# hy-vision-learning/jck-generation

Hardware: AMD Instinct MI355X
Metric: images/sec (G+D step) DCGAN 64x64 bs256 (higher is better)
Workload: dtype bf16; 1 GPU; DCGAN 64x64x3 synthetic, batch 256 per GPU, full G+D step incl. GP pass, RNG and Adam (BASELINE.json configs[1]); per_gpu_batch=256, global_batch=256, parallelism=dp1, dead_D_wgrad_in_G_phase=skipped (never observable: zeroed at train/dcgan_trainer.py:155)

## Files before the change

include/jckgan.h:

```cpp
#ifndef JCKGAN_H
#define JCKGAN_H
#include <stddef.h>
#include <stdint.h>
#ifdef __cplusplus
extern "C" {
#endif

#define JCK_PREC_BF16 0
#define JCK_PREC_F32 1
#define JCK_PREC_BF16X3 2

#define JCK_OK 0
#define JCK_E_ARG (-1)
#define JCK_E_HIP (-2)
#define JCK_E_WS (-3)

const char* jck_last_error(void);
const char* jck_last_launch(void);
const char* jck_launch_name(int i);
int jck_version(void);
int jck_pad_rows(int c);
int jck_pad_chan(int c);

size_t jck_packed_bytes(int prec, long long elems);
int jck_pack_down(int prec, const float* w, int Cs, int Cb, void* wp, void* stream);
int jck_pack_up(int prec, const float* w, int Cs, int Cb, void* wp, void* stream);
int jck_pack_g1(int prec, const float* w, int Ci, int Co, int CiPad, void* wp, void* stream);
int jck_pack_head(const float* w, int C, float* wp, void* stream);

size_t jck_stats_floats(long long pixels, int C, int nyrep);
int jck_conv_down(int prec, const void* big, const void* w, void* small_out, float* stats, int* stats_slots,
                  int N, int Hb, int Wb, int Cb, int Cs, void* stream);
int jck_conv_up(int prec, const void* small_in, const void* w, void* big_out, float* stats, int* stats_slots,
                int epi_tanh, int N, int Hs, int Ws, int Cs, int Cb, void* stream);
size_t jck_conv_wgrad_ws_bytes(int N, int Hb, int Wb, int Cb, int Cs);
int jck_conv_wgrad(int prec, const void* small_side, const void* big_side, float* ws, size_t ws_bytes, float* grad,
                   int accumulate, int N, int Hb, int Wb, int Cb, int Cs, void* stream);
int jck_g1_fwd(int prec, const void* z, const void* w, void* out, float* stats, int* stats_slots, int B, int CiPad,
               int Co, void* stream);
int jck_conv_up_affine(int prec, const void* small_in, const void* w, const float* scale, const float* shift, void* big_out,
                       int N, int Hs, int Ws, int Cs, int Cb, void* stream);
int jck_g1_fwd_affine(int prec, const void* z, const void* w, const float* scale, const float* shift, void* out, int B,
                      int CiPad, int Co, void* stream);
int jck_conv_down_mask(int prec, const void* big, const void* w, const void* a_small, const float* scale, void* small_out,
                       int N, int Hb, int Wb, int Cb, int Cs, void* stream);
int jck_conv_down_affine(int prec, const void* big, const void* w, const float* scale, const float* shift, float slope,
                         void* small_out, int N, int Hb, int Wb, int Cb, int Cs, void* stream);
int jck_latent_loss(int prec, const void* x_nhwc4, const float* target_nchw_f32, void* g_raw_out, float* loss_out, int N, int HW,
                    void* stream);
int jck_latent_adam(int prec, const float* slab, int Z, int ld, float* z, float* m, float* v, float lr, float prior, int t,
                    void* z_operand, int CiPad, int N, void* stream);
int jck_conv_up_mask(int prec, const void* small_in, const void* w, const void* a_big, const float* scale, float slope, void* big_out,
                     int N, int Hs, int Ws, int Cs, int Cb, void* stream);
int jck_leaky_affine_bwd(int prec, const void* g, const void* a, const float* scale, float slope, void* g_y, long long rows, int C,
                         void* stream);
int jck_critic_ds(const float* logit, int mode, float weight, int B, float* ds, float* term, void* stream);
int jck_latent_loss_ex(int prec, const void* x_nhwc4, const float* target_nchw_f32, const float* weight, const void* g_x, void* g_raw_out,
                       float* loss_out, int N, int HW, void* stream);
size_t jck_g1_wgrad_ws_bytes(int B, int CiPad, int Co);
int jck_g1_wgrad(int prec, const void* z, const void* dy, float* ws, size_t ws_bytes, float* grad, int accumulate, int B,
                 int Ci, int CiPad, int Co, void* stream);

int jck_bn_finalize(const float* stats, int slots, float count, const float* gamma, const float* beta,
                    float* running_mean, float* running_var, int64_t* num_batches_tracked, float momentum, float eps,
                    float* aux, int C, void* stream);
int jck_bn_act_fwd(int prec, const void* y, const float* aux, float slope, void* a, long long rows, int C, void* stream);
int jck_bn_eval_aux(int nlayers, const float* const* gamma, const float* const* beta, const float* const* running_mean,
                    const float* const* running_var, float* const* aux, const int* C, float eps, void* stream);
size_t jck_bn_bwd_ws_floats(int C);
int jck_bn_act_bwd(int prec, const void* g_a, const void* y, const float* aux, float slope, float* sums, void* g_y,
                   float* dgamma, float* dbeta, long long rows, int C, void* stream);
int jck_bn_finalize_grouped(const float* stats, int slots_per_group, float count, const float* gamma, const float* beta, float eps,
                            float* aux, float* stat_out, int C, int groups, void* stream);
int jck_bn_fwd(int prec, const void* y, const float* stats, int slots_per_group, float count, const float* gamma, const float* beta,
               float eps, float slope, void* a, float* aux, float* stat_out, float* running_mean, float* running_var, int64_t* nbt,
               float momentum, long long rows_per_group, int C, int groups, void* stream);
int jck_bn_act_fwd_grouped(int prec, const void* y, const float* aux, float slope, void* a, long long rows_per_group, int C,
                           int groups, void* stream);
int jck_bn_act_bwd_grouped(int prec, const void* g_a, const void* y, const float* aux, float slope, float* sums, void* g_y,
                           float* dgamma, float* dbeta, long long rows_per_group, int C, int groups, int grad_groups, void* stream);
size_t jck_grid_sync_bytes(void);
int jck_grid_sync_error(const void* sync_ws);
int jck_bn_act_bwd_res(int prec, const void* g_a, const void* y, const float* aux, float slope, float* sums, void* g_y,
                       float* dgamma, float* dbeta, long long rows_per_group, int C, int groups, int grad_groups, void* sync_ws,
                       void* stream);
int jck_conv_down_grouped(int prec, const void* big, const void* w, void* small_out, float* stats, int* stats_slots, int N, int Hb,
                          int Wb, int Cb, int Cs, int group_images, void* stream);
int jck_conv_up_grouped(int prec, const void* small_in, const void* w, void* big_out, float* stats, int* stats_slots, int N, int Hs,
                        int Ws, int Cs, int Cb, int group_images, void* stream);
int jck_img_prep(int prec, const float* img_nchw, const float* noise_nchw, float keep, float mix, void* out, int N, int HW,
                 void* stream);
int jck_img_prep_u8(int prec, const unsigned char* data, const int64_t* idx, const float* noise, float keep, float mix,
                    void* out_nhwc4, float* out_nchw, int B, int Hs, int Ws, void* stream);
int jck_resize_norm(const float* in, float* out, int N, int C, int H, int W, int OH, int OW, float pre_scale, float pre_shift,
                    const float* mean, const float* stdv, void* stream);
int jck_nhwc4_to_nchw(int prec, const void* in, float* out_nchw, int N, int HW, void* stream);
int jck_img_to_u8(int prec, const void* in, unsigned char* out_u8_nhwc, int N, int HW, void* stream);
int jck_axpy_noise(int prec, const void* x, const float* noise_nchw, float keep, float mix, void* out, int N, int HW,
                   void* stream);
int jck_interp(int prec, const void* a, const void* b, const float* alpha, void* out, int N, int HW, void* stream);
int jck_mix_interp(int prec, const void* x, const float* noise_nchw, const unsigned* rng, int tensor_id, float keep, float mix, void* out,
                   const void* real, const float* alpha, void* xhat, int N, int HW, void* stream);
int jck_gp_norm(int prec, const void* g, int N, int HW, float* scal, int slot, int scal_ld, float* norms, void* stream);
int jck_tanh_bwd(int prec, const void* g, const void* y, float scale, void* out, long long numel, void* stream);
int jck_head_fwd(int prec, const void* a4, const float* wp, const float* bias , int B, int K,
                 float target, int mode, float* prob, float* ds, float* scal, int slot_loss, int slot_p, int scal_ld, void* stream);
int jck_score_head(int prec, const void* x, const float* w, const float* bias , int B, int K,
                   float* logit, float* prob , void* stream);
int jck_head_fwd_grouped(int prec, const void* a4, const float* wp, const float* bias, int B, int K, int G, const float* targets,
                         const int* modes, float* prob, float* ds, float* scal, const int* slot_loss, const int* slot_p,
                         int scal_ld, void* stream);
size_t jck_head_bwd_ws_floats(int K);
int jck_head_bwd(int prec, const float* ds, const float* wp, const void* a4, int B, int K, void* g_a4, float* dwp,
                 int accumulate, float* ws, void* stream);
int jck_head_unpack_grad(const float* dwp, int C, float* grad, int accumulate, void* stream);
int jck_head_bwd_conv(int prec, const float* ds, const float* wp, const void* a4, int B, int C, void* g_a4, float* grad,
                      float* ws, void* stream);
int jck_head_bwd_conv2(int prec, const float* ds, const float* wp, const void* a4, int B, int B_more, int C, void* g_a4, float* grad,
                       float* ws, void* stream);

int jck_pack_linear(int prec, const float* w, int N, int K, int rows, int cols, int transpose, int permC, int permHW, void* wp,
                    void* stream);
int jck_linear_fwd(int prec, const void* x, const void* wp, const float* bias, void* out, int B, int Kpad, int N, int NStore,
                   int ksplit, void* stream);
int jck_linear_finish(int prec, const float* slab, int Z, const float* bias, const float* mask, float scale, void* h, void* hd,
                      int B, int N, void* stream);
size_t jck_linear_wgrad_ws_bytes(int B, int Kpad, int N);
int jck_linear_wgrad(int prec, const void* gy, int ldgy, const void* x, int Kpad, float* ws, size_t ws_bytes, float* gradp,
                     int accumulate, int B, int N, void* stream);
int jck_unperm_linear_grad(const float* gp, int N, int K, int ldp, int permC, int permHW, float* grad, int accumulate, void* stream);
int jck_label_embed_fwd(int prec, const int64_t* labels, const float* W, const float* b, float slope, int B, int NI, int NO,
                        void* cbuf, int ld, int col0, float* pre, void* stream);
int jck_label_embed_bwd(int prec, const void* gc, int ld, int col0, const float* pre, const int64_t* labels, float slope, int B,
                        int NI, int NO, float* dW, float* db, void* stream);
int jck_label_embed_fwd_tiled(int prec, const int64_t* labels, const float* W, const float* b, float slope, int B, int NI, int NO,
                              void* cbuf, int ld, int col0, float* pre, int label_period, void* stream);
int jck_label_embed_bwd_tiled(int prec, const void* gc, int ld, int col0, const float* pre, const int64_t* labels, float slope,
                              int B, int NI, int NO, float* dW, float* db, int label_period, void* stream);
int jck_concat_rows(int prec, const void* a4, int K0, void* cbuf, int ld, int B, void* stream);
int jck_split_rows(int prec, const void* gc, int ld, int K0, void* ga4, int B, void* stream);
int jck_dropout(int prec, const void* x, const float* mask, float scale, void* y, long long n, void* stream);
int jck_colsum(int prec, const void* g, int B, int N, int ld, float* db, void* stream);
int jck_sum_vec(const float* x, int n, float* out, void* stream);
int jck_cgan_z(int prec, const float* z, const int64_t* labels, int B, int NZ, int NL, int CiPad, void* out, void* stream);
int jck_gp_grad(int prec, const void* g, const float* norms, float coef, int N, int HW, void* u, void* stream);
int jck_gp_head2(int prec, const void* ughd, const float* w2, const float* prob, int B, int K, float* rs, float* dw2, float* ws,
                 void* stream);
size_t jck_gp_head2_conv_ws_floats(int B);
int jck_gp_head2_conv(int prec, const void* v4, const void* a4, const float* wp, const float* prob, int B, int C, float* rs,
                      void* g_a4, float* grad, float* ws, void* stream);
size_t jck_bn2_ws_floats(int C);
int jck_bn2_vchain(int prec, const void* v, const void* y, const void* gy, const float* aux, const float* s1, const float* gamma,
                   float slope, float* ws, void* u, void* xdir, float* dgamma, long long rows, int C, void* stream);
int jck_bn2_reverse(int prec, const void* ua, const void* y, const void* xdir, const float* aux, const float* gamma,
                    const float* vsums, float slope, float* ws, void* uy, float* dgamma, float* dbeta, long long rows, int C,
                    void* stream);

int jck_adam(float* p, const float* g, float* m, float* v, long long n, double lr, double beta1, double beta2, double eps,
             int step, float grad_scale, void* stream);
int jck_adam_ema(float* p, const float* g, float* m, float* v, float* ema, long long n, double lr, double beta1, double beta2,
                 double eps, int step, float grad_scale, float ema_weight, const unsigned* skip_if, void* stream);

typedef struct jck_engine jck_engine;
int jck_engine_create(jck_engine** out, int family, int prec, int batch);
int jck_engine_create_sized(jck_engine** out, int family, int prec, int batch, int image_size);
#define JCK_ENGINE_GP_BACKWARD 1u
int jck_engine_create_ex(jck_engine** out, int family, int prec, int batch, int image_size, unsigned flags);
int jck_engine_image_size(const jck_engine*);
int jck_engine_num_tensors_of(const jck_engine*, int net);
int jck_engine_tensor_info_of(const jck_engine*, int net, int idx, char* name, int name_cap, int* kind, long long* offset,
                              long long* numel, int* shape4);
long long jck_engine_arena_numel_of(const jck_engine*, int net, int which);
void jck_engine_destroy(jck_engine*);
int jck_engine_num_tensors(int family, int net );
int jck_engine_tensor_info(int family, int net, int idx, char* name, int name_cap, int* kind, long long* offset,
                           long long* numel, int* shape4);
size_t jck_engine_workspace_bytes(const jck_engine*);
long long jck_engine_arena_numel(int family, int net, int which );
int jck_engine_bind(jck_engine*, void* workspace, size_t ws_bytes, float* g_params, float* g_grads, float* g_m, float* g_v,
                    float* g_bn, int64_t* g_nbt, float* d_params, float* d_grads, float* d_m, float* d_v, float* d_bn,
                    int64_t* d_nbt);
int jck_engine_repack(jck_engine*, int net, void* stream);
#define JCK_PHASE_D_LOSS 0
#define JCK_PHASE_D_GP 1
#define JCK_PHASE_D_STEP 2
#define JCK_PHASE_G_LOSS 3
// ... 109 lines not shown
```

jck-generation_amd/csrc/engine.hip:

```cpp
#include <cstdlib>
#include <cstring>
#include <vector>

#include "ops_internal.hpp"
#include "ew_optim.hpp"
#define JCK_BATCHED_DEFAULT 3
struct jck_engine;
#define TT (e->T)

namespace {

struct TensorInfo { const char* name; int kind; long long offset, numel; int shape[4]; };

struct NetLayout {
  std::vector<TensorInfo> t;
  long long n_params = 0, n_bn = 0;
};

constexpr long long ALIGN_F = 64;

void add_param(NetLayout& L, const char* name, int a, int b, int c, int d) {
  TensorInfo ti{name, 0, L.n_params, (long long)a * b * c * d, {a, b, c, d}};
  L.t.push_back(ti);
  L.n_params = (L.n_params + ti.numel + ALIGN_F - 1) / ALIGN_F * ALIGN_F;
// ... 19 lines not shown
Topo make_topo(int S) {
  Topo T = {};
  T.S = S; T.NS = S == 128 ? 5 : 4; T.HW = S * S;
  T.G_C1 = 64 << (T.NS - 1);
  T.FEAT = 16 * T.G_C1;
  for (int i = 0; i < T.NS; ++i) {
    T.D_CS[i] = 64 << i; T.D_CB[i] = i == 0 ? 3 : 32 << i; T.D_HB[i] = S >> i;
    T.G_CS[i] = T.G_C1 >> i; T.G_CB[i] = i == T.NS - 1 ? 3 : T.G_C1 >> (i + 1); T.G_HS[i] = 4 << i;
  }
  return T;
}
const int N_CLASS = 100, EMB = 200, L1_OUT = 256, L1_FEAT = 8192, L1_K = L1_FEAT + EMB, L1_KPAD = 8448;
constexpr int L1_KSPLIT = 12;
inline int z_dim(int family) { return family == 1 ? 200 : 100; }
inline int z_pad(int family) { return family == 1 ? 256 : 128; }

static const char* const CWN[6] = {"conv1.weight", "conv2.weight", "conv3.weight", "conv4.weight", "conv5.weight", "conv6.weight"};
static const char* const NWN[5] = {"norm1.weight", "norm2.weight", "norm3.weight", "norm4.weight", "norm5.weight"};
static const char* const NBN[5] = {"norm1.bias", "norm2.bias", "norm3.bias", "norm4.bias", "norm5.bias"};
static const char* const RMN[5] = {"norm1.running_mean", "norm2.running_mean", "norm3.running_mean", "norm4.running_mean", "norm5.running_mean"};
static const char* const RVN[5] = {"norm1.running_var", "norm2.running_var", "norm3.running_var", "norm4.running_var", "norm5.running_var"};

NetLayout make_layout(int family, int net, int S = 64) {
  NetLayout L;
  const Topo T = make_topo(S);
  const char* const* CW = CWN; const char* const* NW = NWN; const char* const* NB = NBN; const char* const* RM = RMN; const char* const* RV = RVN;
  if (net == 0) {
    add_param(L, CW[0], z_dim(family), T.G_C1, 4, 4);
    add_bn(L, NW[0], NB[0], RM[0], RV[0], T.G_C1);
    for (int i = 0; i < T.NS; ++i) {
      add_param(L, CW[i + 1], T.G_CS[i], T.G_CB[i], 4, 4);
      if (i < T.NS - 1) add_bn(L, NW[i + 1], NB[i + 1], RM[i + 1], RV[i + 1], T.G_CB[i]);
    }
  } else {
    if (family == 1) {
      add_param(L, "label_embedding.weight", EMB, N_CLASS, 1, 1);
      add_param(L, "label_embedding.bias", EMB, 1, 1, 1);
    }
    for (int i = 0; i < T.NS; ++i) {
      add_param(L, CW[i], T.D_CS[i], T.D_CB[i], 4, 4);
      add_bn(L, NW[i], NB[i], RM[i], RV[i], T.D_CS[i]);
    }
    if (family == 0) {
      add_param(L, CW[T.NS], 1, T.G_C1, 4, 4);
    } else {
      add_param(L, "linear1.weight", L1_OUT, L1_K, 1, 1);
      add_param(L, "linear1.bias", L1_OUT, 1, 1, 1);
      add_param(L, "linear2.weight", 1, L1_OUT, 1, 1);
      add_param(L, "linear2.bias", 1, 1, 1, 1);
    }
  }
  return L;
}

const TensorInfo* find(const NetLayout& L, const char* name) {
  for (auto& t : L.t) if (!strcmp(t.name, name)) return &t;
  return nullptr;
}

struct Carver {
  size_t off = 0;
  unsigned char* base = nullptr;
  template <typename T> T* take(size_t count) {
    T* p = base ? reinterpret_cast<T*>(base + off) : nullptr;
    off = (off + count * sizeof(T) + 255) / 256 * 256;
    return p;
  }
};

struct BnBuf { float *stats, *sums, *aux; int slots; };

struct DActs {
  void *y[JCK_MAX_STAGES], *a[JCK_MAX_STAGES], *g[JCK_MAX_STAGES], *gx;
  float *stats[JCK_MAX_STAGES], *aux[JCK_MAX_STAGES], *sums[JCK_MAX_STAGES], *prob, *ds, *norms;
  int cap, g0, groups;
  DActs group(const jck_engine* e, int first, int n) const;
};

}

static unsigned jck_event_flags() { return hipEventDisableTiming | hipEventDisableSystemFence; }
struct StepState {
  bool gp_done = false;
  bool gp_inflight = false;
  bool join_pending = false, mid_recorded = false;
  long long real_fwd_step = -1;
  bool tail_on_side = false, pre_on_side = false;
  int head_row0 = 0;
  int head_wrow0 = 0;
  int acc_clean_step = -1;
  int dg_clean_step = -1, gg_clean_step = -1;
  long long gz_step = -1;
  void drop_promises() { acc_clean_step = dg_clean_step = gg_clean_step = -1; join_pending = mid_recorded = false; }
  void begin_gp_only() { acc_clean_step = dg_clean_step = -1; gp_done = gp_inflight = false; head_row0 = head_wrow0 = 0; }
};
struct jck_engine {
  int family, prec, B;
  Topo T;
  size_t esz;
  NetLayout LG, LD;
  size_t ws_bytes = 0;
  bool bound = false;
  float *gp = nullptr, *gg = nullptr, *gm = nullptr, *gv = nullptr, *gbn = nullptr;
  float *dp = nullptr, *dg = nullptr, *dm = nullptr, *dv = nullptr, *dbn = nullptr;
  int64_t *gnbt = nullptr, *dnbt = nullptr;
  float* gema = nullptr;
  double ema_decay = 0.0; int ema_start = 0;
  float ema_w(int step) const { return !gema ? 0.f : (step < ema_start ? 1.f : (float)(1.0 - ema_decay)); }
  int graph_nodes = 0;
  void *d_down[JCK_MAX_STAGES], *d_up[JCK_MAX_STAGES];
  float *d_head_wp, *d_head_dwp;
  void *g1_w, *g_up[JCK_MAX_STAGES], *g_down[JCK_MAX_STAGES];
  DActs dset[3] = {};
  DActs bset = {};
  int batched = 0;
  StepState ss;
  float* d_rs[JCK_MAX_STAGES];
  int parity = 0;
  hipStream_t sA = nullptr, sB = nullptr, sC = nullptr;
  hipEvent_t evW[JCK_MAX_STAGES] = {}, evWdone = nullptr, evWmid = nullptr, evHead = nullptr, evTail = nullptr, ev0 = nullptr, evF = nullptr, evReal = nullptr, evGP = nullptr;
  template <typename F> void for_each_side_stream(F f) { for (hipStream_t* p : {&sA, &sB, &sC}) f(*p); }
  template <typename F> void for_each_event(F f) {
    for (hipEvent_t* p : {&evWdone, &evWmid, &evHead, &evTail, &ev0, &evF, &evReal, &evGP}) f(*p);
    for (hipEvent_t& p : evW) f(p);
  }
  bool overlap = true, defer_join = true;
  bool wgrad_side = true;
  bool head_side = true;
  bool ext_events = true;
  unsigned* gsync = nullptr; bool bn_res = true;
  bool cbuf_direct = true;
  bool head_fuse = true;
  bool real_side = true;
  bool fold_zero = true;
  bool fuse_tanh = true;
  void *g_z, *g_y[JCK_MAX_STAGES], *g_a[JCK_MAX_STAGES], *g_gr[JCK_MAX_STAGES], *fake_raw, *fake, *g_raw;
  void *real_noisy, *xhat;
  BnBuf g_bn[JCK_MAX_STAGES];
  float *acc, *scal_out;
  float *acc2, *scal2;
  int acc_ld = 0;
  float *head_ws, *gp2_ws;
  float* hp2;
  unsigned long long noise_seed = 0x6a636b67616e0001ull;
  float *rz[2] = {nullptr, nullptr}, *ralpha[2] = {nullptr, nullptr}, *rmask[2] = {nullptr, nullptr};
  int hp_step[2] = {0, 0};
  float hp_lr[2] = {-1.f, -1.f};
  bool hp_holds(int step, float lr) const { return hp_step[step & 1] == step && hp_lr[step & 1] == lr; }
  bool capturing = false;
  bool gp_bwd = false;
  float* g1_ws = nullptr; size_t g1_ws_bytes = 0;
  float* wg_ws; size_t wg_ws_bytes;
  void *l1_w, *l1_wT;
  void *cbuf, *cbuf2;
  void *h_pre, *h_drop, *g_h, *g_hd, *gh_b1, *ughd, *gc;
  float *pre_e, *l1_slab, *gw1p, *rs, *prob_gp;
  void *d_v[JCK_MAX_STAGES], *d_xdir[JCK_MAX_STAGES], *d_u0;
  float* bn2_ws[JCK_MAX_STAGES]; float* bn2_ws_rev;
  const int64_t* cur_labels = nullptr;
  void* lat_w = nullptr; float *lat_slab = nullptr, *lat_loss = nullptr;
  struct ScoreBufs {
    void* base = nullptr;
    void *x = nullptr, *y = nullptr, *a[JCK_MAX_STAGES] = {}, *cbuf = nullptr, *h = nullptr;
    float *aux[JCK_MAX_STAGES] = {}, *slab = nullptr;
  } sc;
  struct CriticBufs {
    void* base = nullptr;
    void *g[JCK_MAX_STAGES] = {}, *gx = nullptr, *g_h = nullptr, *gc = nullptr;
    float *ds = nullptr, *term = nullptr, *logit = nullptr;
  } cr;
  bool d_packed = false;

  void carve(unsigned char* base) {
    jck_engine* e = this;
    Carver c; c.base = base;
    auto bytes = [&](size_t n) { return n * esz; };
    for (int i = 0; i < TT.NS; ++i) {
      d_down[i] = c.take<unsigned char>(bytes((size_t)jck_pad_rows(TT.D_CS[i]) * 16 * jck_pad_chan(TT.D_CB[i])));
      d_up[i] = c.take<unsigned char>(bytes((size_t)4 * jck_pad_rows(TT.D_CB[i]) * 4 * TT.D_CS[i]));
    }
    d_head_wp = c.take<float>(TT.FEAT); d_head_dwp = c.take<float>(TT.FEAT);
    g1_w = c.take<unsigned char>(bytes((size_t)16 * TT.G_C1 * z_pad(family)));
    for (int i = 0; i < TT.NS; ++i) {
      g_up[i] = c.take<unsigned char>(bytes((size_t)4 * jck_pad_rows(TT.G_CB[i]) * 4 * TT.G_CS[i]));
      g_down[i] = c.take<unsigned char>(bytes((size_t)jck_pad_rows(TT.G_CS[i]) * 16 * jck_pad_chan(TT.G_CB[i])));
    }
    const size_t img = (size_t)B * TT.HW * 4;
    auto take_set = [&](DActs& D, int cap, bool penalty_out) {
      D.cap = D.groups = cap; D.g0 = 0;
      for (int i = 0; i < TT.NS; ++i) {
        const size_t n = (size_t)cap * B * (TT.D_HB[i] / 2) * (TT.D_HB[i] / 2) * TT.D_CS[i];
        D.y[i] = c.take<unsigned char>(bytes(n)); D.a[i] = c.take<unsigned char>(bytes(n)); D.g[i] = c.take<unsigned char>(bytes(n));
        D.sums[i] = c.take<float>(cap * jck_bn_bwd_ws_floats(TT.D_CS[i]));
        D.aux[i] = c.take<float>(cap * 4 * TT.D_CS[i]);
        D.stats[i] = c.take<float>(jck_stats_floats((long long)cap * B * (TT.D_HB[i] / 2) * (TT.D_HB[i] / 2), TT.D_CS[i], 1));
      }
      if (penalty_out) D.gx = c.take<unsigned char>(bytes(img));
      D.prob = c.take<float>((size_t)cap * B); D.ds = c.take<float>((size_t)cap * B);
      if (penalty_out) D.norms = c.take<float>(B);
    };
    for (DActs& D : dset) take_set(D, 1, true);
    for (int i = 0; i < TT.NS; ++i) d_rs[i] = c.take<float>(2 * 4 * 2 * TT.D_CS[i]);
    g_z = c.take<unsigned char>(bytes((size_t)B * z_pad(family)));
    for (int i = 0; i < TT.NS; ++i) {
      const int h = 4 << i, C = TT.G_C1 >> i;
      const size_t n = (size_t)B * h * h * C;
      g_y[i] = c.take<unsigned char>(bytes(n)); g_a[i] = c.take<unsigned char>(bytes(n)); g_gr[i] = c.take<unsigned char>(bytes(n));
    }
    fake_raw = c.take<unsigned char>(bytes(img)); g_raw = c.take<unsigned char>(bytes(img));
    real_noisy = c.take<unsigned char>(bytes(img)); fake = c.take<unsigned char>(bytes(img)); xhat = c.take<unsigned char>(bytes(img));
    if (batched) {
      take_set(bset, 3, false);
      bset.gx = dset[0].gx; bset.norms = dset[0].norms;
    }
    for (int i = 0; i < TT.NS; ++i) g_bn[i].sums = c.take<float>(jck_bn_bwd_ws_floats(TT.G_C1 >> i));
    for (int i = 0; i < TT.NS; ++i) {
      const int C = TT.G_C1 >> i, h = 4 << i;
      g_bn[i].aux = c.take<float>(4 * C);
      g_bn[i].stats = c.take<float>(jck_stats_floats((long long)B * h * h, C, i == 0 ? 16 : 1));
    }
    acc_ld = (B + 63) / 64 * 64;
    acc2 = c.take<float>((size_t)2 * 8 * acc_ld); scal2 = c.take<float>(16);
    acc = acc2; scal_out = scal2;
    hp2 = c.take<float>(16);
    for (int q = 0; q < 2; ++q) {
      rz[q] = c.take<float>((size_t)B * 100); ralpha[q] = c.take<float>((size_t)(B + 3) / 4 * 4);
      rmask[q] = family == 1 ? c.take<float>((size_t)4 * B * L1_OUT) : nullptr;
    }
    head_ws = c.take<float>(jck_head_bwd_ws_floats(TT.FEAT));
    gp2_ws = c.take<float>((size_t)acc_ld + jck_head_bwd_ws_floats(L1_OUT));
    gsync = c.take<unsigned>(jck_grid_sync_bytes() / sizeof(unsigned));
    size_t w = 0;
    for (int i = 0; i < TT.NS; ++i) {
      w = std::max(w, jck_conv_wgrad_ws_bytes(B, TT.D_HB[i], TT.D_HB[i], TT.D_CB[i], TT.D_CS[i]));
      w = std::max(w, jck_conv_wgrad_ws_bytes(2 * B, TT.D_HB[i], TT.D_HB[i], TT.D_CB[i], TT.D_CS[i]));
      w = std::max(w, jck_conv_wgrad_ws_bytes(B, TT.G_HS[i] * 2, TT.G_HS[i] * 2, TT.G_CB[i], TT.G_CS[i]));
    }
    w = std::max(w, jck_g1_wgrad_ws_bytes(B, z_pad(family), TT.G_C1));
    if (family == 1) w = std::max(std::max(w, jck_linear_wgrad_ws_bytes(B, L1_KPAD, L1_OUT)), jck_linear_wgrad_ws_bytes(2 * B, L1_KPAD, L1_OUT));
    wg_ws_bytes = w;
    wg_ws = c.take<float>(w / 4);
    g1_ws_bytes = jck_g1_wgrad_ws_bytes(B, z_pad(family), TT.G_C1);
    g1_ws = c.take<float>(g1_ws_bytes / 4);
    if (family == 1) {
      l1_w = c.take<unsigned char>(bytes((size_t)L1_OUT * L1_KPAD)); l1_wT = c.take<unsigned char>(bytes((size_t)L1_KPAD * L1_OUT));
      const size_t HR = batched ? 3 : 1;
      cbuf = c.take<unsigned char>(bytes(HR * B * L1_KPAD)); cbuf2 = c.take<unsigned char>(bytes((size_t)B * L1_KPAD));
      h_pre = c.take<unsigned char>(bytes(HR * B * L1_OUT)); h_drop = c.take<unsigned char>(bytes(HR * B * L1_OUT));
      g_h = c.take<unsigned char>(bytes(HR * B * L1_OUT)); g_hd = c.take<unsigned char>(bytes(HR * B * L1_OUT));
      gh_b1 = c.take<unsigned char>(bytes((size_t)B * L1_OUT)); ughd = c.take<unsigned char>(bytes((size_t)B * L1_OUT));
      gc = c.take<unsigned char>(bytes(HR * B * L1_KPAD));
      pre_e = c.take<float>(HR * B * EMB); l1_slab = c.take<float>((size_t)L1_KSPLIT * HR * B * L1_OUT);
      gw1p = c.take<float>((size_t)L1_OUT * L1_KPAD);
    }
    if (family == 1 || gp_bwd) {
      rs = c.take<float>(B); prob_gp = c.take<float>(B);
      for (int i = 0; i < TT.NS; ++i) {
        const size_t n = (size_t)B * (TT.D_HB[i] / 2) * (TT.D_HB[i] / 2) * TT.D_CS[i];
        d_v[i] = c.take<unsigned char>(bytes(n)); d_xdir[i] = c.take<unsigned char>(bytes(n));
        bn2_ws[i] = c.take<float>(jck_bn2_ws_floats(TT.D_CS[i]));
      }
      bn2_ws_rev = c.take<float>(jck_bn2_ws_floats(TT.G_C1));
      d_u0 = c.take<unsigned char>(bytes(img));
    }
    ws_bytes = c.off;
  }

  float* P(const NetLayout& L, float* arena, const char* name) const { return arena + find(L, name)->offset; }
  const unsigned* rng() const { return reinterpret_cast<const unsigned*>(hp2 + 8 * parity + 4); }
  int mix_fake_noise(const jck_step_inputs* in, int B, hipStream_t st) {
    if (!in->noise_fake) return jck_axpy_noise_rng(prec, fake_raw, rng(), 1, 0.9f, 0.1f, fake, B, T.HW, st);
    return jck_axpy_noise(prec, fake_raw, in->noise_fake, 0.9f, 0.1f, fake, B, T.HW, st);
  }
  int mix_fake_noise_interp(const jck_step_inputs* in, int B, hipStream_t st) {
    return jck_mix_interp(prec, fake_raw, in->noise_fake, in->noise_fake ? nullptr : rng(), 1, 0.9f, 0.1f, fake, real_noisy, in->alpha, xhat,
                          B, T.HW, st);
  }
};


DActs DActs::group(const jck_engine* e, int first, int n) const {
  DActs v = *this;
  v.g0 = g0 + first; v.groups = n;
  const size_t B = (size_t)e->B;
  auto at = [&](void* p, size_t elems) { return (void*)((unsigned char*)p + elems * e->esz); };
  for (int i = 0; i < TT.NS; ++i) {
    const int cs = TT.D_CS[i];
    const size_t px = (size_t)(TT.D_HB[i] / 2) * (TT.D_HB[i] / 2), off = first * B * px * cs;
    v.y[i] = at(y[i], off); v.a[i] = at(a[i], off); v.g[i] = at(g[i], off);
    v.aux[i] = aux[i] + (size_t)first * 4 * cs;
    v.sums[i] = sums[i] + (size_t)first * jck_bn_bwd_ws_floats(cs);
    v.stats[i] = stats[i] + (size_t)first * (jck_stats_floats((long long)(cap * B * px), cs, 1) / cap / (2 * cs)) * (2 * cs);
  }
  v.prob = prob + first * B; v.ds = ds + first * B;
  return v;
}

static bool env_on(const char* name) {
  const char* v = getenv(name);
  return !(v && atoi(v) == 0);
}
static int create_side_streams(jck_engine* e) {
  hipError_t rc = hipSuccess;
  e->for_each_side_stream([&](hipStream_t& s) { if (rc == hipSuccess) rc = hipStreamCreateWithFlags(&s, hipStreamNonBlocking); });
  e->for_each_event([&](hipEvent_t& ev) { if (rc == hipSuccess) rc = hipEventCreateWithFlags(&ev, jck_event_flags()); });
  HIPCHK(rc);
// ... 215 lines not shown
  return JCK_OK;
}

static int d_head(jck_engine* e, DActs& D, int B, float target, int mode, int slot_loss, int slot_p, hipStream_t st, void* g_out = nullptr) {
  if (e->family == 0)
    return head_fwd_grouped_ev(e->prec, D.a[TT.NS - 1], e->d_head_wp, nullptr, B, TT.FEAT, 1, &target, &mode, D.prob, D.ds, e->acc, &slot_loss,
                               &slot_p, e->acc_ld, g_out, st, nullptr);
  return jck_head_fwd(e->prec, e->h_drop, e->P(e->LD, e->dp, "linear2.weight"), e->P(e->LD, e->dp, "linear2.bias"), B, L1_OUT, target,
                      mode, D.prob, D.ds, e->acc, slot_loss, slot_p, e->acc_ld, st);
}

static int d_head_backward(jck_engine* e, DActs& D, const float* ds, int B, bool want_wgrad, const float* drop_mask, void* ga4_out, hipStream_t st,
                           hipStream_t side = nullptr, bool mid_done = false) {
  if (e->family == 0)
    return jck_head_bwd_conv(e->prec, ds, e->d_head_wp, D.a[TT.NS - 1], B, TT.G_C1, mid_done ? nullptr : ga4_out,
                             want_wgrad ? e->P(e->LD, e->dg, CWN[TT.NS]) : nullptr, e->head_ws, st);
  const size_t r0 = (size_t)e->ss.head_row0, w0 = (size_t)e->ss.head_wrow0;
  auto hb = [&](void* p, size_t row, size_t per_row) { return (void*)((unsigned char*)p + row * per_row * e->esz); };
  void *h_drop = hb(e->h_drop, r0, L1_OUT), *cbuf = hb(e->cbuf, r0, L1_KPAD);
  void *g_hd = hb(e->g_hd, w0, L1_OUT), *g_h = hb(e->g_h, w0, L1_OUT), *gc = hb(e->gc, w0, L1_KPAD);
  const float* pre_e = e->pre_e + r0 * EMB;
  hipStream_t ws = st;
  auto fork = [&](int k) { return fork_side(e, k, st, side, &ws); };
  const float* w2 = e->P(e->LD, e->dp, "linear2.weight");
  if (!mid_done) JCK_TRY(jck_head_bwd(e->prec, ds, w2, h_drop, B, L1_OUT, g_hd, nullptr, 1, e->head_ws, st));
  if (want_wgrad) {
    JCK_TRY(fork(0));
    JCK_TRY(jck_head_bwd(e->prec, ds, w2, h_drop, B, L1_OUT, nullptr, e->P(e->LD, e->dg, "linear2.weight"), 1, e->head_ws, ws));
    JCK_TRY(jck_sum_vec(ds, B, e->P(e->LD, e->dg, "linear2.bias"), ws));
  }
  if (!mid_done) JCK_TRY(jck_dropout(e->prec, g_hd, drop_mask, 1.0f / 0.75f, g_h, (long long)B * L1_OUT, st));
  if (want_wgrad) {
    JCK_TRY(fork(1));
    JCK_TRY(jck_linear_wgrad(e->prec, g_h, L1_OUT, cbuf, L1_KPAD, e->wg_ws, e->wg_ws_bytes, e->gw1p, 1, B, L1_OUT, ws));
    JCK_TRY(jck_colsum(e->prec, g_h, B, L1_OUT, L1_OUT, e->P(e->LD, e->dg, "linear1.bias"), ws));
  }
  JCK_TRY(jck_linear_fwd(e->prec, g_h, e->l1_wT, nullptr, gc, B, L1_OUT, L1_KPAD, L1_KPAD, 1, st));
  if (want_wgrad) {
    JCK_TRY(fork(2));
    JCK_TRY(jck_label_embed_bwd(e->prec, gc, L1_KPAD, TT.FEAT, pre_e, e->cur_labels, LRELU, B, N_CLASS, EMB,
                                e->P(e->LD, e->dg, "label_embedding.weight"), e->P(e->LD, e->dg, "label_embedding.bias"), ws));
  }
  return jck_split_rows(e->prec, gc, L1_KPAD, TT.FEAT, ga4_out, B, st);
}

static int cg_head_backward_batched(jck_engine* e, const float* ds, int B, const float* drop_mask, void* ga4_out, hipStream_t st,
                                    hipStream_t side = nullptr, bool mid_done = false) {
  const int R3 = 3 * B, R2 = 2 * B;
  const float* w2 = e->P(e->LD, e->dp, "linear2.weight");
  hipStream_t ws = st;
  auto fork = [&](int k) { return fork_side(e, k, st, side, &ws); };
  if (!mid_done) JCK_TRY(jck_head_bwd(e->prec, ds, w2, e->h_drop, R3, L1_OUT, e->g_hd, nullptr, 1, e->head_ws, st));
  if (!mid_done) {
    JCK_TRY(fork(0));
    JCK_TRY(jck_head_bwd(e->prec, ds, w2, e->h_drop, R2, L1_OUT, nullptr, e->P(e->LD, e->dg, "linear2.weight"), 1, e->head_ws, ws));
    JCK_TRY(jck_sum_vec(ds, R2, e->P(e->LD, e->dg, "linear2.bias"), ws));
    JCK_TRY(jck_dropout(e->prec, e->g_hd, drop_mask, 1.0f / 0.75f, e->g_h, (long long)R3 * L1_OUT, st));
  }
  JCK_TRY(fork(1));
  if (mid_done) {
    JCK_TRY(jck_head_bwd(e->prec, ds, w2, e->h_drop, R2, L1_OUT, nullptr, e->P(e->LD, e->dg, "linear2.weight"), 1, e->head_ws, ws));
    JCK_TRY(jck_sum_vec(ds, R2, e->P(e->LD, e->dg, "linear2.bias"), ws));
  }
  JCK_TRY(jck_linear_wgrad(e->prec, e->g_h, L1_OUT, e->cbuf, L1_KPAD, e->wg_ws, e->wg_ws_bytes, e->gw1p, 1, R2, L1_OUT, ws));
  JCK_TRY(jck_colsum(e->prec, e->g_h, R2, L1_OUT, L1_OUT, e->P(e->LD, e->dg, "linear1.bias"), ws));
  JCK_TRY(jck_linear_fwd(e->prec, e->g_h, e->l1_wT, nullptr, e->gc, R3, L1_OUT, L1_KPAD, L1_KPAD, 1, st));
  JCK_TRY(fork(2));
  JCK_TRY(jck_label_embed_bwd_tiled(e->prec, e->gc, L1_KPAD, TT.FEAT, e->pre_e, e->cur_labels, LRELU, R2, N_CLASS, EMB,
                                    e->P(e->LD, e->dg, "label_embedding.weight"), e->P(e->LD, e->dg, "label_embedding.bias"), B, ws));
  if (side) HIPCHK(hipEventRecord(e->evHead, side));
  return jck_split_rows(e->prec, e->gc, L1_KPAD, TT.FEAT, ga4_out, R3, st);
}

struct XgradEpi { const void* tanh_y; float scale; void* out; hipEvent_t done; bool fused; };
struct DBackward {
  int gw = 1;
  hipStream_t side = nullptr;
  bool join = true, lazy_join = false;
  int part = 0;
  bool resident = true;
  bool xgrad = false;
  XgradEpi* xe = nullptr;
  bool gp_norm = false;
};
static int d_convs_backward(jck_engine* e, const DActs& S, const void* x_in, int B, hipStream_t st, const DBackward& o) {
  const int G = S.groups, gw = o.gw;
  hipStream_t side = gw > 0 ? o.side : nullptr;
  for (int i = TT.NS - 1; i >= 0; --i) {
    const int hb = TT.D_HB[i], cs = TT.D_CS[i], cb = TT.D_CB[i];
    const long long rows = (long long)B * (hb / 2) * (hb / 2);
    const bool resume = o.part == 2 && i == TT.NS - 1;
    const bool split0 = !resume && i == 0 && e->bn_res && e->prec == JCK_PREC_BF16 && gw > 0 && gw < G;
    hipEvent_t done = side && e->ext_events && !resume ? e->evW[i] : nullptr;
    if (!resume)
      JCK_TRY(bn_act_bwd_res_ev(e->prec, S.g[i], S.y[i], S.aux[i], LRELU, S.sums[i], S.g[i], gw ? e->P(e->LD, e->dg, NWN[i]) : nullptr,
                                gw ? e->P(e->LD, e->dg, NBN[i]) : nullptr, rows, cs, split0 ? gw : G, gw,
                                e->bn_res && o.resident ? e->gsync : nullptr, st, done));
    if (!resume && gw) {
      hipStream_t ws;
      JCK_TRY(fork_side(e, i, st, side, &ws, !done));
      JCK_TRY(jck_conv_wgrad(e->prec, S.g[i], i == 0 ? x_in : S.a[i - 1], e->wg_ws, e->wg_ws_bytes, e->P(e->LD, e->dg, CWN[i]), 1, gw * B, hb, hb, cb,
                             cs, ws));
    }
    if (split0) {
      const DActs P = S.group(e, gw, G - gw);
      JCK_TRY(bn_act_bwd_res_ev(e->prec, P.g[i], P.y[i], P.aux[i], LRELU, P.sums[i], P.g[i], nullptr, nullptr, rows, cs, G - gw, 0, e->gsync, st, nullptr));
    }
    if (o.part == 1) {
      HIPCHK(hipEventRecord(e->evTail, side ? side : st));
      e->ss.tail_on_side = side != nullptr;
      if (side && !o.lazy_join) HIPCHK(hipStreamWaitEvent(st, e->evTail, 0));
      return JCK_OK;
    }
    if (i > 0)
      JCK_TRY(jck_conv_up(e->prec, S.g[i], e->d_up[i], S.g[i - 1], nullptr, nullptr, 0, G * B, hb / 2, hb / 2, cs, cb, st));
    else if (o.xgrad) {
      const void* g0 = S.group(e, G - 1, 1).g[0];
      if (o.xe) JCK_TRY(conv_up_tanh_bwd_ev(e->prec, g0, e->d_up[0], o.xe->tanh_y, o.xe->scale, o.xe->out, B, hb / 2, hb / 2, cs, cb, st, o.xe->done, &o.xe->fused));
      if (!o.xe || !o.xe->fused) JCK_TRY(jck_conv_up(e->prec, g0, e->d_up[0], S.gx, nullptr, nullptr, 0, B, hb / 2, hb / 2, cs, cb, st));
    }
  }
  if (o.gp_norm) JCK_TRY(jck_gp_norm(e->prec, S.gx, B, TT.HW, e->acc, 6, e->acc_ld, S.norms, st));
  if (side && o.join) {
    HIPCHK(hipEventRecord(e->evWdone, side));
    if (o.lazy_join) { e->ss.join_pending = true; e->ss.mid_recorded = false; }
    else HIPCHK(hipStreamWaitEvent(st, e->evWdone, 0));
  }
  return JCK_OK;
}
static int d_backward(jck_engine* e, DActs& D, const void* x_in, int B, const float* drop_mask, hipStream_t st, const DBackward& o,
                      bool head_mid_done = false) {
  JCK_TRY(d_head_backward(e, D, D.ds, B, o.gw > 0, drop_mask, D.g[TT.NS - 1], st, nullptr, head_mid_done));
  return d_convs_backward(e, D, x_in, B, st, o);
}

static int d_batched_pass(jck_engine* e, const void* x_in, int B, int G, const float* targets, const int* slot_loss, const int* slot_p,
                          hipStream_t st, hipStream_t side, int part = 0, bool lazy_tail = false) {
  const DActs S = e->bset.group(e, 0, G);
  const int gw = G - 1;
  DBackward bw;
  bw.gw = gw; bw.side = side; bw.xgrad = bw.gp_norm = true; bw.part = part; bw.lazy_join = part == 1 && lazy_tail;
  if (part == 2) return d_convs_backward(e, S, x_in, B, st, bw);
  {
    float tg[4] = {0.f, 0.f, 0.f, 0.f};
    int md[4] = {0, 0, 0, 0}, sl[4] = {-1, -1, -1, -1}, sp[4] = {-1, -1, -1, -1};
    for (int g = 0; g < G; ++g) {
      const bool pen = g == G - 1;
      tg[g] = pen ? 0.f : targets[g]; md[g] = pen ? 1 : 0; sl[g] = pen ? -1 : slot_loss[g]; sp[g] = pen ? -1 : slot_p[g];
    }
    JCK_TRY(head_fwd_grouped_ev(e->prec, S.a[TT.NS - 1], e->d_head_wp, nullptr, B, TT.FEAT, G, tg, md, S.prob, S.ds, e->acc, sl, sp, e->acc_ld,
                                e->head_fuse ? S.g[TT.NS - 1] : nullptr, st, e->head_fuse && side && e->ext_events ? e->evHead : nullptr));
  }
  const bool hs = side && e->ext_events && e->head_side;
  if (e->head_fuse) {
    const bool hf = side && e->ext_events;
    JCK_TRY(head_bwd_conv2_ev(e->prec, S.ds, e->d_head_wp, S.a[TT.NS - 1], gw * B, 0, TT.G_C1, nullptr, e->P(e->LD, e->dg, CWN[TT.NS]),
                              e->head_ws, st, hf ? side : nullptr, hf ? e->evHead : nullptr));
  } else
    JCK_TRY(head_bwd_conv2_ev(e->prec, S.ds, e->d_head_wp, S.a[TT.NS - 1], gw * B, B, TT.G_C1, S.g[TT.NS - 1], e->P(e->LD, e->dg, CWN[TT.NS]),
                              e->head_ws, st, hs ? side : nullptr, hs ? e->evHead : nullptr));
  return d_convs_backward(e, S, x_in, B, st, bw);
}

static int gp_double_backward(jck_engine* e, const DActs& P, const void* xhat, int B, float lambda, const float* drop_mask, hipStream_t st,
                              hipStream_t side = nullptr, bool lazy_join = false) {
  const size_t esz = e->esz;
  hipStream_t ws = st;
  auto fork = [&](int k) { return fork_side(e, k, st, side, &ws); };
  auto join = [&]() {
    if (!side) return;
    (void)hipEventRecord(e->evWdone, side);
    (void)hipStreamWaitEvent(st, e->evWdone, 0);
  };
  const bool cg = e->family == 1;
  const void* gh1 = e->gh_b1;
  const float* prob1 = e->prob_gp;
  if (cg) {
    if (side) (void)hipStreamWaitEvent(st, e->evHead, 0);
    if (e->ss.head_row0 > 0) {
      gh1 = (const unsigned char*)e->g_h + (size_t)e->ss.head_row0 * L1_OUT * esz;
      prob1 = P.prob;
    } else {
      HIPCHK(hipMemcpyAsync(e->gh_b1, e->g_h, (size_t)B * L1_OUT * esz, hipMemcpyDeviceToDevice, st));
      HIPCHK(hipMemcpyAsync(e->prob_gp, P.prob, (size_t)B * sizeof(float), hipMemcpyDeviceToDevice, st));
    }
  }
  JCK_TRY(jck_gp_grad(e->prec, P.gx, P.norms, 2.0f * lambda / (float)B, B, TT.HW, e->d_u0, st));
  const void* u = e->d_u0;
  for (int i = 0; i < TT.NS; ++i) {
    const int hb = TT.D_HB[i], cs = TT.D_CS[i], cb = TT.D_CB[i];
    const long long rows = (long long)B * (hb / 2) * (hb / 2);
    JCK_TRY(fork(i));
    JCK_TRY(jck_conv_wgrad(e->prec, P.g[i], u, e->wg_ws, e->wg_ws_bytes, e->P(e->LD, e->dg, CWN[i]), 1, B, hb, hb, cb, cs, ws));
    JCK_TRY(jck_conv_down(e->prec, u, e->d_down[i], e->d_v[i], nullptr, nullptr, B, hb, hb, cb, cs, st));
    JCK_TRY(jck_bn2_vchain(e->prec, e->d_v[i], P.y[i], P.g[i], P.aux[i], P.sums[i], e->P(e->LD, e->dp, NWN[i]),
                           LRELU, e->bn2_ws[i], e->d_v[i], e->d_xdir[i], e->P(e->LD, e->dg, NWN[i]), rows, cs, st));
    u = e->d_v[i];
  }
  if (!cg) {
    if (side) (void)hipEventRecord(e->evGP, side);
    JCK_TRY(jck_gp_head2_conv(e->prec, e->d_v[TT.NS - 1], P.a[TT.NS - 1], e->d_head_wp, P.prob, B, TT.G_C1, e->rs, e->d_v[TT.NS - 1],
                              e->P(e->LD, e->dg, CWN[TT.NS]), e->gp2_ws, st));
    if (side) (void)hipStreamWaitEvent(st, e->evGP, 0);
  } else {
    JCK_TRY(jck_concat_rows(e->prec, e->d_v[TT.NS - 1], TT.FEAT, e->cbuf2, L1_KPAD, B, st));
    JCK_TRY(fork(0));
    JCK_TRY(jck_linear_wgrad(e->prec, gh1, L1_OUT, e->cbuf2, L1_KPAD, e->wg_ws, e->wg_ws_bytes, e->gw1p, 1, B, L1_OUT, ws));
    if (side) (void)hipEventRecord(e->evGP, side);
    JCK_TRY(jck_linear_fwd(e->prec, e->cbuf2, e->l1_w, nullptr, e->l1_slab, B, L1_KPAD, L1_OUT, L1_OUT, L1_KSPLIT, st));
    const bool fuse = e->head_fuse && L1_OUT == 256;
    if (!fuse) JCK_TRY(jck_linear_finish(e->prec, e->l1_slab, L1_KSPLIT, nullptr, drop_mask, 1.0f / 0.75f, nullptr, e->ughd, B, L1_OUT, st));
    hipStream_t hs = e->head_side && e->ext_events ? side : nullptr;
    if (fuse) {
      const size_t w0 = (size_t)e->ss.head_wrow0 * L1_OUT * esz;
      JCK_TRY(gp_head_mid_ev(e->prec, e->l1_slab, L1_KSPLIT, drop_mask, 1.0f / 0.75f, e->ughd, e->P(e->LD, e->dp, "linear2.weight"), prob1, B, e->rs,
                             e->P(e->LD, e->dg, "linear2.weight"), e->gp2_ws, (unsigned char*)e->g_hd + w0, (unsigned char*)e->g_h + w0, st, hs,
                             hs ? e->evHead : nullptr));
    } else
      JCK_TRY(gp_head2_ev(e->prec, e->ughd, e->P(e->LD, e->dp, "linear2.weight"), prob1, B, L1_OUT, e->rs,
                          e->P(e->LD, e->dg, "linear2.weight"), e->gp2_ws, st, hs, hs ? e->evHead : nullptr));
    if (side) (void)hipStreamWaitEvent(st, e->evGP, 0); else join();
    JCK_TRY(d_head_backward(e, e->dset[0], e->rs, B, true, drop_mask, e->d_v[TT.NS - 1], st, hs, fuse));
    JCK_TRY(jck_unperm_linear_grad(e->gw1p, L1_OUT, L1_K, L1_KPAD, 512, 16, e->P(e->LD, e->dg, "linear1.weight"), 1, hs ? hs : st));
  }
// ... 304 lines not shown
  HIPCHK(hipMemsetAsync(e->acc, 0, (size_t)8 * e->acc_ld * sizeof(float), c.st));
  HIPCHK(hipMemsetAsync(e->dg, 0, e->LD.n_params * sizeof(float), c.st));
  if (c.cg) HIPCHK(hipMemsetAsync(e->gw1p, 0, (size_t)L1_OUT * L1_KPAD * sizeof(float), c.st));
  e->ss.begin_gp_only();
  JCK_TRY(jck_img_prep(e->prec, c.in->real_nchw, nullptr, 1.0f, 0.0f, e->real_noisy, c.B, c.HW, c.st));
  JCK_TRY(jck_img_prep(e->prec, c.in->noise_real, nullptr, 1.0f, 0.0f, e->fake, c.B, c.HW, c.st));
  JCK_TRY(penalty_pass(e, c, c.D0, c.st));
  if (c.cg || e->gp_bwd) JCK_TRY(gp_double_backward(e, c.D0, e->xhat, c.B, 1.0f, c.in->drop_mask[2], c.st, nullptr));
  return JCK_OK;
}

static int phase_d_gp(jck_engine* e, const PhaseCtx& c) {
  if (!c.in->alpha) JCK_FAIL(JCK_E_ARG, "PHASE_D_GP needs alpha");
  if (e->ss.gp_done && (c.cg || e->gp_bwd)) {
    e->ss.gp_done = false;
    JCK_TRY(gp_double_backward(e, e->bset.group(e, 2, 1), e->xhat, c.B, 10.0f, c.in->drop_mask[2], c.st, c.sA, c.lazy));
    if (!(c.lazy && c.sA)) e->ss.join_pending = e->ss.mid_recorded = false;
    e->ss.head_row0 = 0;
    return JCK_OK;
  }
  if (e->ss.gp_done) { e->ss.gp_done = false; return JCK_OK; }
  if (e->ss.gp_inflight) {
    HIPCHK(hipStreamWaitEvent(c.st, e->evGP, 0));
    e->ss.gp_inflight = false;
    if (e->gp_bwd) JCK_TRY(gp_double_backward(e, c.D1, e->xhat, c.B, 10.0f, nullptr, c.st, c.sA));
    return JCK_OK;
  }
  JCK_TRY(penalty_pass(e, c, c.D0, c.st));
  if (c.cg || e->gp_bwd) JCK_TRY(gp_double_backward(e, c.D0, e->xhat, c.B, 10.0f, c.in->drop_mask[2], c.st, c.sA));
  return JCK_OK;
}

static int phase_d_step(jck_engine* e, const PhaseCtx& c) {
  if (e->ss.gp_inflight || (e->gp_bwd && e->ss.gp_done)) JCK_FAIL(JCK_E_ARG, "PHASE_D_GP must be called before PHASE_D_STEP");
  if (!e->hp_holds(c.in->step, c.in->lr) && !e->capturing) JCK_TRY(refresh_adam_scalars(e, c.in->step, c.in->lr, c.st));
  const float* hp = e->hp2 + 8 * e->parity;
  float* zg = (e->fold_zero && !e->capturing && e->LG.n_params % 4 == 0) ? e->gg : nullptr;
  if (zg) e->ss.gg_clean_step = c.in->step;
  if (e->ss.join_pending) {
    const TensorInfo* c1 = find(e->LD, CWN[0]);
    const long long cut = c1->offset + c1->numel;
    HIPCHK(hipStreamWaitEvent(c.st, e->ss.mid_recorded ? e->evWmid : e->evWdone, 0));
    JCK_TRY(adam_net(e, 1, cut, e->LD.n_params - cut, c.in->grad_scale, hp, c.st, zg));
    JCK_TRY(repack_linear(e, c.st));
    if (e->ss.mid_recorded) HIPCHK(hipStreamWaitEvent(c.st, e->evWdone, 0));
    e->ss.join_pending = e->ss.mid_recorded = false;
    JCK_TRY(adam_net(e, 1, 0, cut, c.in->grad_scale, hp, c.st));
    return repack_convs(e, 1, c.st);
  }
  JCK_TRY(adam_net(e, 1, 0, e->LD.n_params, c.in->grad_scale, hp, c.st, zg));
  return jck_engine_repack(e, 1, c.st);
}

static int phase_g_loss(jck_engine* e, const PhaseCtx& c) {
  JCK_TRY(clear_or_memset(e, e->ss.gg_clean_step, c.in->step, c.st, e->gg, e->LG.n_params * sizeof(float)));
  const bool fuse = e->head_fuse;
  JCK_TRY(d_forward(e, c.D0, e->fake, c.B, 3, c.in->drop_mask[3], c.st, !fuse));
  if (fuse && !c.cg) JCK_TRY(d_head(e, c.D0, c.B, 0.9f, 0, 2, 5, c.st, c.D0.g[TT.NS - 1]));
  else if (fuse) {
    const float tg1 = 0.9f;
    const int md1 = 0, sl1 = 2, sp1 = 5;
    JCK_TRY(cg_head_middle(e, c.B, 1, &tg1, &md1, &sl1, &sp1, c.D0.prob, c.D0.ds, c.in->drop_mask[3], c.st));
  } else JCK_TRY(d_head(e, c.D0, c.B, 0.9f, 0, 2, 5, c.st));
  XgradEpi xe = {e->fake_raw, 0.9f, e->g_raw, (c.sA && e->ext_events) ? e->evW[TT.NS - 1] : nullptr, false};
  DBackward bw;
  bw.gw = 0; bw.xgrad = true; bw.xe = e->fuse_tanh ? &xe : nullptr;
  JCK_TRY(d_backward(e, c.D0, e->fake, c.B, c.in->drop_mask[3], c.st, bw, fuse));
  return g_backward(e, c.D0.gx, c.B, c.st, c.sA, xe.fused);
}

static int phase_g_step(jck_engine* e, const PhaseCtx& c) {
  if (!e->hp_holds(c.in->step, c.in->lr) && !e->capturing) JCK_TRY(refresh_adam_scalars(e, c.in->step, c.in->lr, c.st));
  JCK_TRY(adam_net(e, 0, 0, e->LG.n_params, c.in->grad_scale, e->hp2 + 8 * e->parity, c.st, nullptr, e->gema));
  TailJobs t = {};
  for (int i = 0; i < TT.NS; ++i) {
    const int cs = TT.D_CS[i];
    t.l[i].rec = e->d_rs[i] + (size_t)e->parity * 4 * 2 * cs;
    t.l[i].rm = e->dbn + find(e->LD, RMN[i])->offset;
    t.l[i].rv = e->dbn + find(e->LD, RVN[i])->offset;
    t.l[i].nbt = (long long*)(e->dnbt + i);
    t.l[i].C = cs;
  }
  t.nl = TT.NS; t.npass = 4; t.momentum = BN_MOM; t.acc = e->acc; t.acc_ld = e->acc_ld; t.B = c.B; t.invB = 1.0f / (float)c.B; t.lambda_gp = 10.0f; t.out = e->scal_out;
  return repack_convs(e, 0, c.st, &t, cdiv(TT.G_C1, 256));
}

static int phase_begin(jck_engine* e, int phase, jck_step_inputs& loc, hipStream_t st) {
  const bool cg = e->family == 1;
  const int q = loc.step & 1;
  if (!loc.z) loc.z = e->rz[q];
  if (!loc.alpha) loc.alpha = e->ralpha[q];
  if (cg && !loc.drop_mask[0] && !loc.drop_mask[1] && !loc.drop_mask[2] && !loc.drop_mask[3])
    for (int i = 0; i < 4; ++i) loc.drop_mask[i] = e->rmask[q] + (size_t)i * e->B * L1_OUT;
  if (e->ss.join_pending && !(phase == JCK_PHASE_D_STEP || (phase == JCK_PHASE_D_GP && cg && e->ss.gp_done))) {
    HIPCHK(hipStreamWaitEvent(st, e->evWdone, 0));
    e->ss.join_pending = e->ss.mid_recorded = false;
  }
  if (cg) {
    if (!loc.labels) JCK_FAIL(JCK_E_ARG, "CGAN phases need labels");
    e->cur_labels = loc.labels;
  }
  e->parity = q;
  if (!e->capturing) {
    const int ph = phase & 0xff;
    const bool zero_d = ph == JCK_PHASE_D_LOSS || ph == JCK_PHASE_D_LOSS_A || ph == JCK_PHASE_D_REAL || ph == JCK_PHASE_D_REAL_FWD;
    if (e->hp_step[q] != loc.step) JCK_TRY(set_step_impl(e, loc.step, loc.lr, st, zero_d));
    else if (e->hp_lr[q] != loc.lr) JCK_TRY(refresh_adam_scalars(e, loc.step, loc.lr, st));
  }
  e->acc = e->acc2 + (size_t)8 * e->acc_ld * e->parity;
  e->scal_out = e->scal2 + 8 * e->parity;
  return JCK_OK;
}
static int phase_impl(jck_engine* e, int phase, const jck_step_inputs* in_, void* stream) {
  if (!e || !e->bound || !in_) JCK_FAIL(JCK_E_ARG, "engine not bound / null inputs");
  hipStream_t st = (hipStream_t)stream;
  const bool cg = e->family == 1;
  const bool lazy = (phase & JCK_PHASE_LAZY_JOIN) && cg && !e->capturing;
  const bool lazy_tail = (phase & JCK_PHASE_LAZY_JOIN) && !cg && (phase & 0xff) == JCK_PHASE_D_LOSS_A;
  phase &= ~JCK_PHASE_LAZY_JOIN;
  jck_step_inputs loc = *in_;
  JCK_TRY(phase_begin(e, phase, loc, st));
  const bool par = e->overlap && !e->capturing;
  const PhaseCtx c = {st, (par && e->wgrad_side) ? e->sA : nullptr, &loc, in_, e->B, TT.HW, cg, lazy, lazy_tail, par, par, par && !cg,
                      cg ? e->dset[0] : e->dset[2], e->dset[0], e->dset[1]};
  switch (phase) {
    case JCK_PHASE_D_LOSS_A: case JCK_PHASE_D_LOSS_B: return phase_d_loss_batched(e, c, phase);
    case JCK_PHASE_D_LOSS: return e->batched ? phase_d_loss_batched(e, c, phase) : phase_d_per_pass(e, c, phase);
    case JCK_PHASE_D_REAL: case JCK_PHASE_D_FAKE: return phase_d_per_pass(e, c, phase);
    case JCK_PHASE_D_REAL_FWD: return phase_d_real_fwd(e, c);
    case JCK_PHASE_GP_ONLY: return phase_gp_only(e, c);
    case JCK_PHASE_D_GP: return phase_d_gp(e, c);
    case JCK_PHASE_D_STEP: return phase_d_step(e, c);
    case JCK_PHASE_G_LOSS: return phase_g_loss(e, c);
    case JCK_PHASE_G_STEP: return phase_g_step(e, c);
  }
  JCK_FAIL(JCK_E_ARG, "unknown phase");
}
extern "C" int jck_engine_phase(jck_engine* e, int phase, const jck_step_inputs* in_, void* stream) {
  const bool keep_res = e ? e->bn_res : false;
  if (e && (phase & JCK_PHASE_NO_RESIDENT)) e->bn_res = false;
  const int rc = phase_impl(e, phase & ~JCK_PHASE_NO_RESIDENT, in_, stream);
  if (e) e->bn_res = keep_res;
  if (rc != JCK_OK && e) {
    if (e->ss.join_pending && e->sA && stream && !e->capturing) (void)hipStreamWaitEvent((hipStream_t)stream, e->evWdone, 0);
    e->ss.drop_promises();
  }
  return rc;
}

static int set_step_impl(jck_engine* e, int step, float lr, void* stream, bool zero_d) {
  if (!e || !e->bound) JCK_FAIL(JCK_E_ARG, "engine not bound");
  if (e->capturing) JCK_FAIL(JCK_E_ARG, "set_step inside a graph capture would bake one step's scalars into the graph");
  const int q = step & 1;
  zero_d = zero_d && e->fold_zero && e->LD.n_params % 4 == 0;
  JCK_TRY(jck_adam_set_step(e->hp2 + 8 * q, (double)lr, ADAM_B1, ADAM_B2, step, e->noise_seed, e->ema_w(step), (hipStream_t)stream, e->rz[q], (long long)e->B * 100,
                            e->ralpha[q], e->B, e->rmask[q], e->rmask[q] ? (long long)4 * e->B * L1_OUT : 0, 0.75f,
                            e->acc2 + (size_t)8 * e->acc_ld * q, (long long)8 * e->acc_ld,
                            zero_d ? e->dg : nullptr, e->LD.n_params, zero_d && e->family == 1 ? e->gw1p : nullptr, (long long)L1_OUT * L1_KPAD,
                            e->family == 0 && e->fold_zero ? e->g_z : nullptr, 100, z_pad(e->family), prec_f32_storage(e->prec) ? 1 : 0));
  e->ss.gz_step = (e->family == 0 && e->fold_zero) ? step : -1;
  if (zero_d) e->ss.dg_clean_step = step;
  e->ss.acc_clean_step = step;
  e->hp_step[step & 1] = step;
  e->hp_lr[step & 1] = lr;
  return JCK_OK;
}
extern "C" int jck_engine_set_step(jck_engine* e, int step, float lr, void* stream) { return set_step_impl(e, step, lr, stream, false); }
extern "C" int jck_engine_bind_ema(jck_engine* e, float* g_ema) {
  if (!e || !e->bound) JCK_FAIL(JCK_E_ARG, "engine not bound");
  if (e->capturing) JCK_FAIL(JCK_E_ARG, "bind_ema inside a graph capture");
  if ((uintptr_t)g_ema & 15) JCK_FAIL(JCK_E_ARG, "bind_ema: the EMA arena must be 16-byte aligned");
  e->gema = g_ema;
  e->hp_step[0] = e->hp_step[1] = 0;
  e->hp_lr[0] = e->hp_lr[1] = -1.f;
  return JCK_OK;
}
extern "C" int jck_engine_set_ema(jck_engine* e, double decay, int start_step) {
  if (!e) JCK_FAIL(JCK_E_ARG, "null engine");
  if (!(decay >= 0.0 && decay <= 1.0)) JCK_FAIL(JCK_E_ARG, "set_ema: decay must lie in [0, 1]");
  e->ema_decay = decay; e->ema_start = start_step;
  e->hp_step[0] = e->hp_step[1] = 0;
  e->hp_lr[0] = e->hp_lr[1] = -1.f;
  return JCK_OK;
}
extern "C" int jck_engine_set_noise_seed(jck_engine* e, unsigned long long seed) {
  if (!e) JCK_FAIL(JCK_E_ARG, "null engine");
  e->noise_seed = seed;
  e->hp_step[0] = e->hp_step[1] = 0;
  e->hp_lr[0] = e->hp_lr[1] = -1.f;
  return JCK_OK;
}

// ... 288 lines not shown
  if (!e || !e->bound) JCK_FAIL(JCK_E_ARG, w + ": engine not bound");
  if (n < 1 || n > e->B) JCK_FAIL(JCK_E_ARG, w + ": n must be in [1, batch]");
  if (!z) JCK_FAIL(JCK_E_ARG, w + ": null z");
  if (critic_mode < 0 || critic_mode > 2) JCK_FAIL(JCK_E_ARG, w + ": critic_mode must be 0 (none), 1 (nsgan) or 2 (logit)");
  if (!target && !critic_mode) JCK_FAIL(JCK_E_ARG, w + ": without a target a critic is required");
  if (!(critic_weight >= 0.f)) JCK_FAIL(JCK_E_ARG, w + ": critic_weight >= 0");
  if (e->family == 1 && !labels) JCK_FAIL(JCK_E_ARG, w + ": CGAN needs labels");
  if (critic_mode && !e->d_packed)
    JCK_FAIL(JCK_E_ARG, w + ": the discriminator's weights were never packed (load a discriminator state and repack net 1 first)");
  if (e->capturing) JCK_FAIL(JCK_E_ARG, w + ": not inside a graph capture");
  return JCK_OK;
}
struct LatentEx { const float* target; const float* weight; int mode; float cw; const int64_t* labels; };
static int latent_ex_begin(jck_engine* e, const LatentEx& o, hipStream_t st) {
  if (!o.mode) return JCK_OK;
  JCK_TRY(score_alloc(e, st));
  JCK_TRY(critic_alloc(e));
  return score_fold(e, st);
}
static int latent_eval_ex(jck_engine* e, const LatentEx& o, int n, float* loss, float* term, float* logit, hipStream_t st) {
  if (!o.weight && !o.mode) return latent_eval(e, o.target, n, loss, st);
  JCK_TRY(g_eval_products(e, n, st));
  const jck_engine::ScoreBufs& S = e->sc;
  const jck_engine::CriticBufs& C = e->cr;
  if (o.mode) {
    const int top = TT.NS - 1;
    if (!logit) logit = C.logit;
    JCK_TRY(score_stages_head(e, e->fake_raw, o.labels, n, logit, nullptr, st));
    JCK_TRY(jck_critic_ds(logit, o.mode, o.cw, n, C.ds, term ? term : C.term, st));
    if (e->family == 0) {
      JCK_TRY(jck_head_bwd_conv(e->prec, C.ds, e->d_head_wp, S.a[top], n, TT.G_C1, C.g[top], nullptr, nullptr, st));
    } else {
      JCK_TRY(jck_head_bwd(e->prec, C.ds, e->P(e->LD, e->dp, "linear2.weight"), nullptr, n, L1_OUT, C.g_h, nullptr, 0, nullptr, st));
      JCK_TRY(jck_linear_fwd(e->prec, C.g_h, e->l1_wT, nullptr, C.gc, n, L1_OUT, L1_KPAD, L1_KPAD, 1, st));
      JCK_TRY(jck_split_rows(e->prec, C.gc, L1_KPAD, TT.FEAT, C.g[top], n, st));
    }
    JCK_TRY(jck_leaky_affine_bwd(e->prec, C.g[top], S.a[top], S.aux[top], LRELU, C.g[top], (long long)n * (TT.D_HB[top] / 2) * (TT.D_HB[top] / 2),
                                 TT.D_CS[top], st));
    for (int i = top; i >= 1; --i) {
      const int hs = TT.D_HB[i] / 2;
      JCK_TRY(jck_conv_up_mask(e->prec, C.g[i], e->d_up[i], S.a[i - 1], S.aux[i - 1], LRELU, C.g[i - 1], n, hs, hs, TT.D_CS[i], TT.D_CB[i], st));
    }
    JCK_TRY(jck_conv_up(e->prec, C.g[0], e->d_up[0], C.gx, nullptr, nullptr, 0, n, TT.D_HB[0] / 2, TT.D_HB[0] / 2, TT.D_CS[0], TT.D_CB[0], st));
  }
  JCK_TRY(jck_latent_loss_ex(e->prec, e->fake_raw, o.target, o.weight, o.mode ? C.gx : nullptr, e->g_raw, loss, n, TT.HW, st));
  return latent_backward(e, n, st);
}
extern "C" int jck_engine_latent_grad_ex(jck_engine* e, const float* z, const int64_t* labels, const float* target_nchw, const float* weight,
                                         int critic_mode, float critic_weight, int n, float* loss, float* term, float* logit, float* dz,
                                         void* stream) {
  JCK_TRY(latent_ex_check(e, z, labels, target_nchw, critic_mode, critic_weight, n, "latent_grad_ex"));
  if (!loss || !dz) JCK_FAIL(JCK_E_ARG, "latent_grad_ex: null loss / dz");
  hipStream_t st = (hipStream_t)stream;
  const LatentEx o = {target_nchw, weight, critic_mode, critic_weight, labels};
  JCK_TRY(latent_begin(e, z, labels, n, st));
  JCK_TRY(latent_ex_begin(e, o, st));
  JCK_TRY(latent_eval_ex(e, o, n, loss, term, logit, st));
  return jck_latent_adam(e->prec, e->lat_slab, LAT_KSPLIT, LAT_LD, dz, nullptr, nullptr, 0.f, 0.f, 0, nullptr, 0, n, st);
}
extern "C" int jck_engine_project_ex(jck_engine* e, float* z, const int64_t* labels, const float* target_nchw, int n, int steps, float lr,
                                     float prior, const float* weight, int critic_mode, float critic_weight, float* m, float* v, int t0,
                                     float* loss_hist, float* term_hist, void* stream) {
  JCK_TRY(latent_ex_check(e, z, labels, target_nchw, critic_mode, critic_weight, n, "project_ex"));
  if (steps < 1 || t0 < 0 || !m || !v) JCK_FAIL(JCK_E_ARG, "project_ex: steps >= 1, t0 >= 0 and the Adam state m, v are required");
  if (!(lr > 0.f) || !(prior >= 0.f)) JCK_FAIL(JCK_E_ARG, "project_ex: lr > 0 and prior >= 0");
  hipStream_t st = (hipStream_t)stream;
  const LatentEx o = {target_nchw, weight, critic_mode, critic_weight, labels};
  JCK_TRY(latent_begin(e, z, labels, n, st));
  JCK_TRY(latent_ex_begin(e, o, st));
  for (int s = 0; s < steps; ++s) {
    JCK_TRY(latent_eval_ex(e, o, n, loss_hist ? loss_hist + (size_t)s * n : e->lat_loss, term_hist ? term_hist + (size_t)s * n : nullptr, nullptr, st));
    JCK_TRY(jck_latent_adam(e->prec, e->lat_slab, LAT_KSPLIT, LAT_LD, z, m, v, lr, prior, t0 + s + 1, e->g_z, z_pad(e->family), n, st));
  }
  return JCK_OK;
}

extern "C" const void* jck_engine_tensor(const jck_engine* e, const char* name, long long* numel) {
  if (!e || !e->bound || !name) return nullptr;
  const long long img = (long long)e->B * TT.HW * 4;
  const DActs& D = e->dset[0];
  struct { const char* n; const void* p; long long c; } tab[] = {
      {"fake", e->fake, img}, {"fake_raw", e->fake_raw, img}, {"real_noisy", e->real_noisy, img}, {"xhat", e->xhat, img},
      {"d_gx", D.gx, img}, {"prob", D.prob, e->B}, {"ds", D.ds, e->B}, {"norms", D.norms, e->B}, {"acc", e->acc, (long long)8 * e->acc_ld},
      {"d_y1", D.y[0], (long long)e->B * (TT.S / 2) * (TT.S / 2) * 64}, {"d_a4", D.a[TT.NS - 1], (long long)e->B * TT.FEAT},
      {"g_y1", e->g_y[0], (long long)e->B * TT.FEAT}, {"g_a4", e->g_a[TT.NS - 1], (long long)e->B * (TT.S / 2) * (TT.S / 2) * 64}};
  for (auto& t : tab)
    if (!strcmp(t.n, name)) { if (numel) *numel = t.c; return t.p; }
  return nullptr;
}
```

jck-generation_amd/csrc/ew_optim.hpp:

```cpp
#pragma once
#include "common.hpp"
#include "philox.hpp"

struct StepRng { float* z; long long nz; float* alpha; long long nalpha; float* masks; long long nmask; float keep_p; float* zero; long long nzero;
                 float* zbig[2]; long long nzbig[2];
                 void* zpad; int zd, zp, zpad_f32; };
__device__ __forceinline__ float u01(unsigned x) { return ((float)(x >> 8) + 0.5f) * (1.0f / 16777216.0f); }
static __global__ void adam_hp_kernel(float* __restrict__ hp, float step_size, float bc2_sqrt, unsigned seed_lo, unsigned seed_hi,
                                      unsigned step, const StepRng r, float ema_w) {
  if (threadIdx.x == 0 && blockIdx.x == 0) {
    hp[0] = step_size; hp[1] = bc2_sqrt; hp[2] = ema_w;
    unsigned* w = reinterpret_cast<unsigned*>(hp + 4);
    w[0] = seed_lo; w[1] = seed_hi; w[2] = step; w[3] = 0u;
  }
  const long long q0 = (r.nz + 3) / 4, q1 = (r.nalpha + 3) / 4, q2 = (r.nmask + 3) / 4;
  for (long long i = blockIdx.x * (long long)blockDim.x + threadIdx.x; i < r.nzero; i += (long long)gridDim.x * blockDim.x) r.zero[i] = 0.f;
#pragma unroll
  for (int b = 0; b < 2; ++b)
    for (long long i = blockIdx.x * (long long)blockDim.x + threadIdx.x; i < (r.nzbig[b] >> 2); i += (long long)gridDim.x * blockDim.x)
      reinterpret_cast<f32x4*>(r.zbig[b])[i] = f32x4{0.f, 0.f, 0.f, 0.f};
  for (long long i = blockIdx.x * (long long)blockDim.x + threadIdx.x; i < q0 + q1 + q2; i += (long long)gridDim.x * blockDim.x) {
    unsigned o[4];
    if (i < q0) {
      philox4x32_10((unsigned)i, (unsigned)(i >> 32), 8u, step, seed_lo, seed_hi, o);
// ... 151 lines not shown
  if (u >= J.total) return;
  W* wp = reinterpret_cast<W*>(J.wp);
  float v[16];
  auto load16 = [&](const float* src) {
#pragma unroll
    for (int q = 0; q < 4; ++q) {
      const f32x4 t = *reinterpret_cast<const f32x4*>(src + 4 * q);
      v[4 * q] = t[0]; v[4 * q + 1] = t[1]; v[4 * q + 2] = t[2]; v[4 * q + 3] = t[3];
    }
  };
  switch (J.kind) {
    case 0: {
      const int Cb = J.b, cs = (int)(u / Cb), cb = (int)(u % Cb);
      load16(J.w + ((long long)cs * Cb + cb) * 16);
      W* d = wp + (((long long)cs * 16) << J.c) + cb;
#pragma unroll
      for (int t = 0; t < 16; ++t) stf(d + ((long long)t << J.c), v[t]);
    } break;
    case 1: {
      const int Cs = J.a, Cb = J.b, cb = (int)(u / Cs), cs = (int)(u % Cs);
      load16(J.w + ((long long)cs * Cb + cb) * 16);
      const long long K = 4ll * Cs, per = (long long)J.c * K;
#pragma unroll
      for (int phase = 0; phase < 4; ++phase)
#pragma unroll
        for (int t = 0; t < 4; ++t) {
          const int kh = c_up_k[phase >> 1][t >> 1], kw = c_up_k[phase & 1][t & 1];
          stf(wp + phase * per + (long long)cb * K + (long long)t * Cs + cs, v[kh * 4 + kw]);
        }
    } break;
    case 2: {
      const int Cs = J.a, Cb = J.b, c = (int)(u / Cs), cs = (int)(u % Cs);
      load16(J.w + ((long long)cs * Cb + c) * 16);
      const long long K = 9ll * Cs;
#pragma unroll
      for (int phase = 0; phase < 4; ++phase)
#pragma unroll
        for (int t9 = 0; t9 < 9; ++t9) {
          const int dy = t9 / 3 - 1, dx = t9 % 3 - 1, ph = phase >> 1, pw = phase & 1;
          const int kh = ph == 0 ? (dy == 0 ? 1 : (dy == -1 ? 3 : -1)) : (dy == 1 ? 0 : (dy == 0 ? 2 : -1));
          const int kw = pw == 0 ? (dx == 0 ? 1 : (dx == -1 ? 3 : -1)) : (dx == 1 ? 0 : (dx == 0 ? 2 : -1));
          if (kh >= 0 && kw >= 0) stf(wp + (long long)(phase * 4 + c) * K + (long long)t9 * Cs + cs, v[kh * 4 + kw]);
        }
    } break;
    case 3: {
      const int Ci = J.a, Co = J.b, co = (int)(u / Ci), ci = (int)(u % Ci);
      load16(J.w + ((long long)ci * Co + co) * 16);
#pragma unroll
      for (int t = 0; t < 16; ++t) stf(wp + ((long long)t * Co + co) * J.c + ci, v[t]);
    } break;
    default: {
      const int c = (int)u;
      load16(J.w + (long long)c * 16);
#pragma unroll
      for (int t = 0; t < 16; ++t) reinterpret_cast<float*>(J.wp)[(long long)t * J.a + c] = v[t];
    } break;
  }
}
template <typename W>
__global__ __launch_bounds__(256) void pack_multi_kernel(const PackJobs jobs) { pack_multi_block<W>(jobs, (int)blockIdx.x); }

template <typename T>
__global__ void cast_f32_kernel(const float* __restrict__ in, T* __restrict__ out, long long n) {
  for (long long i = blockIdx.x * (long long)blockDim.x + threadIdx.x; i < n; i += (long long)gridDim.x * blockDim.x)
    stf(out + i, in[i]);
}
template <typename T>
__global__ void cast_to_f32_kernel(const T* __restrict__ in, float* __restrict__ out, long long n) {
  for (long long i = blockIdx.x * (long long)blockDim.x + threadIdx.x; i < n; i += (long long)gridDim.x * blockDim.x)
    out[i] = ldf(in + i);
}

template <typename T>
__global__ void pad_rows_kernel(const float* __restrict__ in, int B, int Ci, int CiPad, T* __restrict__ out) {
  const long long total = (long long)B * CiPad;
  for (long long i = blockIdx.x * (long long)blockDim.x + threadIdx.x; i < total; i += (long long)gridDim.x * blockDim.x) {
    const int c = (int)(i % CiPad);
    const long long b = i / CiPad;
    stf(out + i, c < Ci ? in[b * Ci + c] : 0.f);
  }
}

struct TailLayer { const float* rec; float* rm; float* rv; long long* nbt; int C; };
struct TailJobs { TailLayer l[5]; int nl; int npass; float momentum; const float* acc; int acc_ld, B; float invB, lambda_gp; float* out; };
__device__ __forceinline__ void step_tail_block(const TailJobs& t, int bx, int by) {
  if (by == t.nl) {
    if (bx != 0) return;
    __shared__ float sm[4];
    float tot[7];
#pragma unroll
    for (int q = 0; q < 7; ++q) {
      float s = 0.f;
      for (int n = threadIdx.x; n < t.B; n += 256) s += t.acc[(long long)q * t.acc_ld + n];
      tot[q] = block_sum256(s, sm);
    }
    if (threadIdx.x == 0) {
      const float lr = tot[0] * t.invB, lf = tot[1] * t.invB, gp = tot[6] * t.invB;
      t.out[0] = (lr + lf) + t.lambda_gp * gp;
      t.out[1] = tot[2] * t.invB;
      t.out[2] = tot[3] * t.invB;
      t.out[3] = tot[4] * t.invB;
      t.out[4] = tot[5] * t.invB;
      t.out[5] = gp;
      t.out[6] = lr;
      t.out[7] = lf;
    }
    return;
  }
  const TailLayer& L = t.l[by];
  const int c = bx * blockDim.x + threadIdx.x;
  if (c == 0 && L.nbt) *L.nbt += t.npass;
  if (c >= L.C) return;
  float rm = L.rm[c], rv = L.rv[c];
  for (int p = 0; p < t.npass; ++p) {
    rm = (1.f - t.momentum) * rm + t.momentum * L.rec[(long long)p * 2 * L.C + c];
    rv = (1.f - t.momentum) * rv + t.momentum * L.rec[(long long)p * 2 * L.C + L.C + c];
  }
  L.rm[c] = rm;
  L.rv[c] = rv;
}
template <typename W>
__global__ __launch_bounds__(256) void pack_tail_kernel(const PackJobs jobs, int pack_chunks, const TailJobs t, int tail_x) {
  if ((int)blockIdx.x < pack_chunks) { pack_multi_block<W>(jobs, (int)blockIdx.x); return; }
  const int q = (int)blockIdx.x - pack_chunks;
  step_tail_block(t, q % tail_x, q / tail_x);
}
```

jck-generation_amd/csrc/ops_gemm.hip:

```cpp
#include "ops_internal.hpp"
#include "igemm.hpp"
#include "thin.hpp"
#include "wgrad.hpp"

#define DISPATCH_P(prec, CALL)                                          \
  do {                                                                  \
    if ((prec) == JCK_PREC_BF16) { typedef PrecBf16 P; return CALL; }   \
    if ((prec) == JCK_PREC_F32) { typedef PrecF32 P; return CALL; }     \
    if ((prec) == JCK_PREC_BF16X3) { typedef PrecBf16x3 P; return CALL; } \
    JCK_FAIL(JCK_E_ARG, "bad prec");                                    \
  } while (0)

template <auto KERN, int LDS_LIMIT = 0, class Params>
static int launch_lds(dim3 grid, dim3 block, int lds, hipStream_t st, const Params& q) {
  static bool attr_done = false;
  if (!attr_done) {
    HIPCHK(hipFuncSetAttribute(reinterpret_cast<const void*>(KERN), hipFuncAttributeMaxDynamicSharedMemorySize, LDS_LIMIT ? LDS_LIMIT : lds));
    attr_done = true;
  }
  hipLaunchKernelGGL(KERN, grid, block, lds, st, q);
  HIPCHK(hipGetLastError());
  return JCK_OK;
}

// ... 169 lines not shown
}

template <class P>
static int launch_igemm_mask_leaky_p(const IgemmParams& p, int nch_pad, int phases, int nsub, hipStream_t st) {
  if (nsub != 1 || (nch_pad != 64 && nch_pad % 128)) JCK_FAIL(JCK_E_ARG, "igemm: the leaky mask epilogue is built for >= 64 gathered channels and >= 64 output rows");
  if (nch_pad % 128 == 0) {
    const long long wgs = (long long)cdiv(p.M, 128) * (nch_pad / 128) * phases;
    if constexpr (!P::IS_F32) {
      const long long wgs256 = (long long)cdiv(p.M, 256) * (nch_pad / 128) * phases;
      if (wgs256 >= IGEMM_256_MIN_TILES && p.M % 256 == 0) return launch_igemm_dma<128, 256, 3, true, 8, false, true, true>(p, nch_pad, phases, st, nullptr);
      if (wgs >= 512) return launch_igemm_dma<128, 128, 2, false, 4, false, true, true>(p, nch_pad, phases, st, nullptr);
      return launch_igemm_dma<128, 64, 3, true, 4, false, true, true>(p, nch_pad, phases, st, nullptr);
    } else {
      if (wgs >= 256) return launch_igemm_t<P, 128, 128, 1, false, true, true>(p, nch_pad, phases, st, nullptr);
      return launch_igemm_t<P, 128, 64, 1, false, true, true>(p, nch_pad, phases, st, nullptr);
    }
  }
  if constexpr (!P::IS_F32) return launch_igemm_dma<64, 128, 2, false, 4, false, true, true>(p, nch_pad, phases, st, nullptr);
  else return launch_igemm_t<P, 64, 128, 1, false, true, true>(p, nch_pad, phases, st, nullptr);
}

static int launch_wgrad_reduce(const float* ws, int Z, int CsRows, int ncols, int Cs, int Cb, int logCbPad, float* grad,
                               int accumulate, hipStream_t st);
static int launch_igemm(int prec, const IgemmParams& p0, int nch_pad, int phases, int nsub, hipStream_t st, int* slots, bool leaky = false) {
  IgemmParams p = p0;
  for (int zz = 0; zz < 4; ++zz)
    for (int t = 0; t < 16; ++t) p.tap[zz][t] = ((int)p.dy[zz][t] << 16) | ((int)p.dx[zz][t] & 0xffff);
  const long long esz = prec_f32_storage(prec) ? 4 : 2;
  if (nsub == 0 && (p.logC < 3 || p.logC > 5 || !(p.aff_scale || p.mask_act))) JCK_FAIL(JCK_E_ARG, "igemm: 8..32 gathered channels are built for the affine and mask epilogues alone");
  if (nsub == 1 && p.logC < 6 && !p.act_row_elems) JCK_FAIL(JCK_E_ARG, "igemm: the gathered tensor needs >= 64 channels (or exactly 4)");
  {
    const long long nimg = ((long long)p.M + (1ll << p.logOHW) - 1) >> p.logOHW;
    const long long ab = p.act_row_elems ? (long long)p.M * p.act_row_elems * esz : nimg * p.H * p.W * (1ll << p.logC) * esz;
    const long long wb = (long long)(p.ksplit > 1 ? 1 : phases) * (p.w_phase_stride ? p.w_phase_stride : (long long)nch_pad * p.K) * esz;
    if (ab >= (1ll << 31) || wb >= (1ll << 31)) JCK_FAIL(JCK_E_ARG, "igemm: operand exceeds 2 GiB (32-bit buffer offsets)");
    p.act_bytes = (unsigned)ab; p.w_bytes = (unsigned)wb;
  }
  if (p.K % IG_BK != 0) JCK_FAIL(JCK_E_ARG, "igemm: K must be a multiple of 64, got " + std::to_string(p.K));
  if (p.M <= 0) JCK_FAIL(JCK_E_ARG, "igemm: empty problem");
  if (p.stats && !slots) JCK_FAIL(JCK_E_ARG, "igemm: stats requested without a slot-count output");
  if (p.aff_scale) {
    if (!p.aff_shift || p.stats || p.bias || p.epi || p.ksplit > 1 || p.rows_are_phases || !is_pow2(p.cstat) || p.cstat % 4 ||
        ((uintptr_t)p.aff_scale | (uintptr_t)p.aff_shift) % 16)
      JCK_FAIL(JCK_E_ARG, "igemm: the affine epilogue takes 16-byte aligned scale and shift, a power-of-two channel count and no other option");
    if (leaky) DISPATCH_P(prec, (launch_igemm_affine_p<P, true>(p, nch_pad, phases, nsub, st)));
    DISPATCH_P(prec, launch_igemm_affine_p<P>(p, nch_pad, phases, nsub, st));
  }
  if (p.mask_act && leaky) {
    if (!p.mask_scale || p.stats || p.bias || p.epi || p.ksplit > 1 || p.rows_are_phases || !is_pow2(p.cstat) || p.cstat % 4 ||
        (uintptr_t)p.mask_scale % 16 || (uintptr_t)p.mask_act % 16)
      JCK_FAIL(JCK_E_ARG, "igemm: the mask epilogue takes a 16-byte aligned scale and activation, a power-of-two channel count and no other option");
    DISPATCH_P(prec, launch_igemm_mask_leaky_p<P>(p, nch_pad, phases, nsub, st));
  }
  if (p.mask_act) {
    if (!p.mask_scale || p.stats || p.bias || p.epi || p.ksplit > 1 || p.rows_are_phases || phases != 1 || !is_pow2(p.cstat) || p.cstat % 4 ||
        (uintptr_t)p.mask_scale % 16 || (uintptr_t)p.mask_act % 16)
      JCK_FAIL(JCK_E_ARG, "igemm: the mask epilogue takes a 16-byte aligned scale and activation, a power-of-two channel count and no other option");
    DISPATCH_P(prec, launch_igemm_mask_p<P>(p, nch_pad, nsub, st));
  }
  DISPATCH_P(prec, launch_igemm_p<P>(p, nch_pad, phases, nsub, st, slots));
}

#define IMG_GPW 8
static int launch_img_down(const void* x, const void* w, void* out, float* stats, int* slots, int N, int Hb, int Wb, double flops,
                           hipStream_t st) {
  ImgDownParams q = {};
  const int OH = Hb / 2, OW = Wb / 2;
  q.x = x; q.w = w; q.out = out; q.stats = stats;
  q.ngroups = N * OH * (OW / 16); q.H = Hb; q.W = Wb; q.logOH = ilog2(OH); q.logG = ilog2(OW / 16);
  q.x_bytes = (unsigned)((long long)N * Hb * Wb * 4 * 2);
  const int grid = cdiv(q.ngroups, 4 * IMG_GPW);
  if (stats) {
    if (!slots) JCK_FAIL(JCK_E_ARG, "conv_down: stats requested without a slot-count output");
    *slots = grid;
  }
  ProfScope prof(K_IMG_DOWN, flops, st);
  note_launch(K_IMG_DOWN);
  hipLaunchKernelGGL(img_down_kernel<IMG_GPW>, dim3(grid), dim3(256), 0, st, q);
  HIPCHK(hipGetLastError());
  return JCK_OK;
}
#define IMG_UP_R 8
static int launch_img_up(const void* a, const void* w, void* out, int epi_tanh, int N, int Hs, int Ws, double flops, hipStream_t st,
                         const void* mul_t = nullptr, float mul_scale = 1.f, hipEvent_t done = nullptr) {
  ImgUpParams q = {};
  q.a = a; q.w = w; q.out = out; q.epi_tanh = epi_tanh; q.mul_t = mul_t; q.mul_scale = mul_scale;
  q.nunits = N * (Hs / IMG_UP_R) * (Ws / 16); q.Hs = Hs; q.Ws = Ws; q.logYB = ilog2(Hs / IMG_UP_R); q.logG = ilog2(Ws / 16);
  q.a_bytes = (unsigned)((long long)N * Hs * Ws * 64 * 2);
  ProfScope prof(K_IMG_UP, flops, st);
  note_launch(K_IMG_UP);
  LAUNCH_EV(img_up_kernel<IMG_UP_R>, dim3(cdiv(q.nunits, 4)), dim3(256), 0, st, done, q);
  HIPCHK(hipGetLastError());
  return JCK_OK;
}

static int conv_down_impl(int prec, const void* big, const void* w, void* small_out, float* stats, int* stats_slots,
                          int N, int Hb, int Wb, int Cb, int Cs, void* stream, int fwd_group_images = 0,
                          const void* mask_act = nullptr, const float* mask_scale = nullptr, const float* aff_scale = nullptr,
                          const float* aff_shift = nullptr, float aff_slope = 0.f) {
  const int cbp = jck_pad_chan(Cb);
  if (!is_pow2(cbp) || !is_pow2(Hb) || !is_pow2(Wb) || Hb < 2 || Wb < 2 || Cs % 4 != 0)
    JCK_FAIL(JCK_E_ARG, "conv_down: shapes must be powers of two (Hb,Wb,Cb) and Cs % 4 == 0");
  if ((long long)N * Hb * Wb * cbp >= (1ll << 31)) JCK_FAIL(JCK_E_ARG, "conv_down: tensor exceeds 2^31 elements");
  IgemmParams p = {};
  p.act = big; p.w = w; p.out = small_out; p.stats = stats;
  const int OH = Hb / 2, OW = Wb / 2;
  p.M = N * OH * OW; p.NchStore = Cs; p.logC = ilog2(cbp); p.K = 16 << p.logC;
  p.H = Hb; p.W = Wb; p.logOW = ilog2(OW); p.logOHW = ilog2(OH * OW); p.sy = p.sx = 2; p.ntaps = 16;
  for (int t = 0; t < 16; ++t) { p.dy[0][t] = (signed char)(t / 4 - 1); p.dx[0][t] = (signed char)(t % 4 - 1); }
  p.osN = (long long)OH * OW * Cs; p.osY = OW * Cs; p.osX = Cs; p.obase[0] = 0;
  p.cstat = Cs; p.ytiles_per_cset = 1; p.epi = 0; p.w_phase_stride = 0;
  if (stats && !is_pow2(Cs)) JCK_FAIL(JCK_E_ARG, "conv_down: BN statistics need a power-of-two channel count");
  p.flops = 2.0 * p.M * Cs * 16.0 * Cb;
  if (stats && fwd_group_images > 0) { p.bn_group_rows = fwd_group_images * OH * OW; p.stat_accum = 1; }
  p.mask_act = mask_act; p.mask_scale = mask_scale;
  p.aff_scale = aff_scale; p.aff_shift = aff_shift; p.aff_slope = aff_slope;
  if (aff_scale) return launch_igemm(prec, p, jck_pad_rows(Cs), 1, cbp == 4 ? 2 : 1, (hipStream_t)stream, nullptr, true);
  if (!mask_act && prec == JCK_PREC_BF16 && cbp == 4 && Cs == 64 && OW % 16 == 0 && is_pow2(OH))
    return launch_img_down(big, w, small_out, stats, stats_slots, N, Hb, Wb, p.flops, (hipStream_t)stream);
  return launch_igemm(prec, p, jck_pad_rows(Cs), 1, cbp == 4 ? 2 : (mask_act && cbp < 64 ? 0 : 1), (hipStream_t)stream, stats_slots);
}
extern "C" int jck_conv_down_mask(int prec, const void* big, const void* w, const void* a_small, const float* scale, void* small_out,
                                  int N, int Hb, int Wb, int Cb, int Cs, void* stream) {
  if (!a_small || !scale) JCK_FAIL(JCK_E_ARG, "conv_down_mask: the activation and the scale are required");
  if (!is_pow2(Cs)) JCK_FAIL(JCK_E_ARG, "conv_down_mask: Cs must be a power of two");
  return conv_down_impl(prec, big, w, small_out, nullptr, nullptr, N, Hb, Wb, Cb, Cs, stream, 0, a_small, scale);
}
extern "C" int jck_conv_down_affine(int prec, const void* big, const void* w, const float* scale, const float* shift, float slope,
                                    void* small_out, int N, int Hb, int Wb, int Cb, int Cs, void* stream) {
  if (!big || !w || !small_out || !scale || !shift) JCK_FAIL(JCK_E_ARG, "conv_down_affine: null tensor, scale or shift");
  if (N < 1) JCK_FAIL(JCK_E_ARG, "conv_down_affine: N must be >= 1");
  if (!is_pow2(Cs) || Cs < 64) JCK_FAIL(JCK_E_ARG, "conv_down_affine: Cs must be a power of two >= 64");
  if (Cb == 3 || Cb == 4) {
    if (Cs != 64) JCK_FAIL(JCK_E_ARG, "conv_down_affine: a 3 / 4-channel input is built for Cs = 64");
  } else if (Cb < 64 || !is_pow2(Cb)) {
    JCK_FAIL(JCK_E_ARG, "conv_down_affine: Cb must be 3, 4 or a power of two >= 64");
  }
  return conv_down_impl(prec, big, w, small_out, nullptr, nullptr, N, Hb, Wb, Cb, Cs, stream, 0, nullptr, nullptr, scale, shift, slope);
}
extern "C" int jck_conv_down(int prec, const void* big, const void* w, void* small_out, float* stats, int* stats_slots,
                             int N, int Hb, int Wb, int Cb, int Cs, void* stream) {
  return conv_down_impl(prec, big, w, small_out, stats, stats_slots, N, Hb, Wb, Cb, Cs, stream);
}
extern "C" int jck_conv_down_grouped(int prec, const void* big, const void* w, void* small_out, float* stats, int* stats_slots,
                                     int N, int Hb, int Wb, int Cb, int Cs, int group_images, void* stream) {
  if (group_images < 1 || N % group_images) JCK_FAIL(JCK_E_ARG, "conv_down_grouped: N must be a multiple of group_images >= 1");
  return conv_down_impl(prec, big, w, small_out, stats, stats_slots, N, Hb, Wb, Cb, Cs, stream, group_images);
}
static int conv_up_impl(int prec, const void* small_in, const void* w, void* big_out, float* stats, int* stats_slots,
                        int epi_tanh, int N, int Hs, int Ws, int Cs, int Cb, void* stream, int fwd_group_images = 0,
                        const float* aff_scale = nullptr, const float* aff_shift = nullptr, const void* mask_act = nullptr,
                        const float* mask_scale = nullptr, float mask_slope = 0.f) {
  const int cbp = jck_pad_chan(Cb);
  if (aff_scale && (Cb < 8 || !is_pow2(Cb))) JCK_FAIL(JCK_E_ARG, "conv_up_affine: Cb must be a power of two >= 8");
  if (!is_pow2(Cs) || Cs < 16 || !is_pow2(Hs) || !is_pow2(Ws) || cbp % 4 != 0)
    JCK_FAIL(JCK_E_ARG, "conv_up: shapes must be powers of two (Hs,Ws,Cs>=16)");
  if ((long long)N * Hs * Ws * 4 * cbp >= (1ll << 31)) JCK_FAIL(JCK_E_ARG, "conv_up: tensor exceeds 2^31 elements");
  IgemmParams p = {};
  p.act = small_in; p.w = w; p.out = big_out; p.stats = stats;
  p.M = N * Hs * Ws; p.NchStore = cbp; p.logC = ilog2(Cs); p.K = 4 << p.logC;
  p.H = Hs; p.W = Ws; p.logOW = ilog2(Ws); p.logOHW = ilog2(Hs * Ws); p.sy = p.sx = 1; p.ntaps = 4;
  if (cbp == 4) {
    if (Cs % 64) JCK_FAIL(JCK_E_ARG, "conv_up: Cs % 64 != 0 for a <=4-channel output");
    if (stats) JCK_FAIL(JCK_E_ARG, "conv_up: statistics are not provided for <=4-channel outputs");
    p.ntaps = 9; p.K = 9 * Cs; p.NchStore = 16; p.rows_are_phases = 1;
    for (int t = 0; t < 9; ++t) { p.dy[0][t] = (signed char)(t / 3 - 1); p.dx[0][t] = (signed char)(t % 3 - 1); }
    for (int ph = 0; ph < 2; ++ph)
      for (int pw = 0; pw < 2; ++pw) p.obase[ph * 2 + pw] = (ph * 2 * Ws + pw) * cbp;
    p.osN = (long long)4 * Hs * Ws * cbp; p.osY = 2 * 2 * Ws * cbp; p.osX = 2 * cbp;
    p.cstat = 4; p.ytiles_per_cset = 1; p.epi = epi_tanh ? 1 : 0; p.w_phase_stride = 0;
    p.flops = 2.0 * p.M * 4.0 * Cb * 4.0 * Cs;
    if (prec == JCK_PREC_BF16 && Cs == 64 && Ws % 16 == 0 && Hs % IMG_UP_R == 0)
      return launch_img_up(small_in, w, big_out, epi_tanh ? 1 : 0, N, Hs, Ws, p.flops, (hipStream_t)stream);
    return launch_igemm(prec, p, 16, 1, 1, (hipStream_t)stream, nullptr);
  }
  static const int DI[2][2] = {{0, -1}, {1, 0}};
  for (int ph = 0; ph < 2; ++ph)
    for (int pw = 0; pw < 2; ++pw) {
      const int z = ph * 2 + pw;
      for (int t = 0; t < 4; ++t) { p.dy[z][t] = (signed char)DI[ph][t >> 1]; p.dx[z][t] = (signed char)DI[pw][t & 1]; }
      p.obase[z] = (ph * 2 * Ws + pw) * cbp;
    }
  p.osN = (long long)4 * Hs * Ws * cbp; p.osY = 2 * 2 * Ws * cbp; p.osX = 2 * cbp;
  p.cstat = cbp; p.ytiles_per_cset = 1; p.epi = epi_tanh ? 1 : 0;
  if (stats && !is_pow2(cbp)) JCK_FAIL(JCK_E_ARG, "conv_up: BN statistics need a power-of-two channel count");
  const int rows = jck_pad_rows(Cb);
  p.w_phase_stride = (long long)rows * p.K;
  if (p.K % 64 != 0) JCK_FAIL(JCK_E_ARG, "conv_up: 4*Cs must be a multiple of 64");
  p.flops = 2.0 * p.M * 4.0 * Cb * 4.0 * Cs;
  if (stats && fwd_group_images > 0) { p.bn_group_rows = fwd_group_images * Hs * Ws; p.stat_accum = 1; }
  p.aff_scale = aff_scale; p.aff_shift = aff_shift;
  p.mask_act = mask_act; p.mask_scale = mask_scale;
  if (mask_act) { p.aff_slope = mask_slope; return launch_igemm(prec, p, rows, 4, 1, (hipStream_t)stream, nullptr, true); }
  return launch_igemm(prec, p, rows, 4, aff_scale && Cs < 64 ? 0 : 1, (hipStream_t)stream, stats_slots);
}
int conv_up_tanh_bwd_ev(int prec, const void* small_in, const void* w, const void* tanh_y, float scale, void* out, int N, int Hs, int Ws,
                        int Cs, int Cb, hipStream_t stream, hipEvent_t done, bool* fused) {
  *fused = prec == JCK_PREC_BF16 && jck_pad_chan(Cb) == 4 && Cs == 64 && Ws % 16 == 0 && Hs % IMG_UP_R == 0 &&
           is_pow2(Hs) && is_pow2(Ws) && (long long)N * Hs * Ws * 16 < (1ll << 31);
  if (!*fused) return JCK_OK;
  return launch_img_up(small_in, w, out, 0, N, Hs, Ws, 2.0 * N * Hs * Ws * 4.0 * Cb * 4.0 * Cs, stream, tanh_y, scale, done);
}
extern "C" int jck_conv_up(int prec, const void* small_in, const void* w, void* big_out, float* stats, int* stats_slots,
                           int epi_tanh, int N, int Hs, int Ws, int Cs, int Cb, void* stream) {
  return conv_up_impl(prec, small_in, w, big_out, stats, stats_slots, epi_tanh, N, Hs, Ws, Cs, Cb, stream);
}
extern "C" int jck_conv_up_mask(int prec, const void* small_in, const void* w, const void* a_big, const float* scale, float slope,
                                void* big_out, int N, int Hs, int Ws, int Cs, int Cb, void* stream) {
  if (!small_in || !w || !a_big || !scale || !big_out) JCK_FAIL(JCK_E_ARG, "conv_up_mask: null tensor, activation or scale");
  if (N < 1) JCK_FAIL(JCK_E_ARG, "conv_up_mask: N must be >= 1");
  if (!is_pow2(Cs) || Cs < 64 || !is_pow2(Cb) || Cb < 64) JCK_FAIL(JCK_E_ARG, "conv_up_mask: Cs and Cb must be powers of two >= 64");
  if ((uintptr_t)scale % 16 || (uintptr_t)a_big % 16) JCK_FAIL(JCK_E_ARG, "conv_up_mask: the scale and the activation must be 16-byte aligned");
  return conv_up_impl(prec, small_in, w, big_out, nullptr, nullptr, 0, N, Hs, Ws, Cs, Cb, stream, 0, nullptr, nullptr, a_big, scale, slope);
}
extern "C" int jck_conv_up_grouped(int prec, const void* small_in, const void* w, void* big_out, float* stats, int* stats_slots,
                                   int N, int Hs, int Ws, int Cs, int Cb, int group_images, void* stream) {
  if (group_images < 1 || N % group_images) JCK_FAIL(JCK_E_ARG, "conv_up_grouped: N must be a multiple of group_images >= 1");
  return conv_up_impl(prec, small_in, w, big_out, stats, stats_slots, 0, N, Hs, Ws, Cs, Cb, stream, group_images);
}
static int g1_fwd_impl(int prec, const void* z, const void* w, void* out, float* stats, int* stats_slots, int B,
                       int CiPad, int Co, void* stream, const float* aff_scale = nullptr, const float* aff_shift = nullptr) {
  if (!is_pow2(CiPad) || CiPad < 64 || !is_pow2(Co) || (16 * Co) % 128 != 0)
    JCK_FAIL(JCK_E_ARG, "g1_fwd: CiPad must be a power of two >= 64, Co a power of two");
  IgemmParams p = {};
  p.act = z; p.w = w; p.out = out; p.stats = stats;
  p.M = B; p.NchStore = 16 * Co; p.logC = ilog2(CiPad); p.K = CiPad;
  p.H = 1; p.W = 1; p.logOW = 0; p.logOHW = 0; p.sy = p.sx = 1; p.ntaps = 1;
  p.dy[0][0] = 0; p.dx[0][0] = 0;
  p.osN = (long long)16 * Co; p.osY = 0; p.osX = 0; p.obase[0] = 0;
  p.cstat = Co; p.ytiles_per_cset = 1; p.epi = 0; p.w_phase_stride = 0;
  if (Co < 128 && !aff_scale) JCK_FAIL(JCK_E_ARG, "g1_fwd: Co must be >= 128");
  p.flops = 2.0 * B * 16.0 * Co * CiPad;
  p.aff_scale = aff_scale; p.aff_shift = aff_shift;
  return launch_igemm(prec, p, 16 * Co, 1, 1, (hipStream_t)stream, stats_slots);
}
extern "C" int jck_g1_fwd(int prec, const void* z, const void* w, void* out, float* stats, int* stats_slots, int B,
                          int CiPad, int Co, void* stream) {
  return g1_fwd_impl(prec, z, w, out, stats, stats_slots, B, CiPad, Co, stream);
}
extern "C" int jck_conv_up_affine(int prec, const void* small_in, const void* w, const float* scale, const float* shift, void* big_out,
                                  int N, int Hs, int Ws, int Cs, int Cb, void* stream) {
  if (!scale || !shift) JCK_FAIL(JCK_E_ARG, "conv_up_affine: scale and shift are required");
  return conv_up_impl(prec, small_in, w, big_out, nullptr, nullptr, 0, N, Hs, Ws, Cs, Cb, stream, 0, scale, shift);
}
extern "C" int jck_g1_fwd_affine(int prec, const void* z, const void* w, const float* scale, const float* shift, void* out, int B,
                                 int CiPad, int Co, void* stream) {
  if (!scale || !shift) JCK_FAIL(JCK_E_ARG, "g1_fwd_affine: scale and shift are required");
  if (Co < 4) JCK_FAIL(JCK_E_ARG, "g1_fwd_affine: Co must be >= 4");
  return g1_fwd_impl(prec, z, w, out, nullptr, nullptr, B, CiPad, Co, stream, scale, shift);
}

struct WgradPlan { int BG, BS, gx, gy, Z, mchunk, CsRows, ncols; size_t ws; };

constexpr int WGRAD_SMALL_WGS = 512;
static WgradPlan plan_wgrad(long long Mtot, int ncols, int Cs) {
  WgradPlan pl;
  pl.ncols = ncols;
  pl.BG = (ncols % 128 == 0) ? 128 : 64;
  pl.BS = (Cs >= 128) ? 128 : 64;
  pl.gx = cdiv(ncols, pl.BG);
  pl.gy = cdiv(Cs, pl.BS);
  pl.CsRows = pl.gy * pl.BS;
  const int tiles = pl.gx * pl.gy;
  long long Z = std::max(1, (tiles >= 4 ? g_wgrad_wgs : WGRAD_SMALL_WGS) / tiles);
  const long long maxZ = std::max(1ll, Mtot / (WG_BKP * 4));
  Z = std::min(Z, maxZ);
  long long mchunk = (Mtot + Z - 1) / Z;
  mchunk = (mchunk + 63) / 64 * 64;
  Z = (Mtot + mchunk - 1) / mchunk;
  pl.Z = (int)Z; pl.mchunk = (int)mchunk;
  pl.ws = (size_t)Z * pl.CsRows * ncols * sizeof(float);
  return pl;
}

template <class P, int BG, int BS, int NSUB>
static int launch_wgrad_t(const WgradParams& p, const WgradPlan& pl, hipStream_t st) {
  constexpr KernelId id = kid_wgrad<P, BG, BS, NSUB>();
  ProfScope prof(id, p.flops, st);
  note_launch(id);
  constexpr int LDSB = WgradCfg<P, BG, BS>::LDS_BYTES;
  return launch_lds<wgrad_kernel<P, BG, BS, NSUB>>(dim3(pl.gx, pl.gy, pl.Z), dim3(256), LDSB, st, p);
}

template <int NSTG, bool WS>
static int launch_wgrad_dma_t(const WgradParams& q, int grid, hipStream_t st) {
  constexpr int LDSB = NSTG * 2 * WGD_BKP * 256;
  ProfScope prof(WS ? K_WGRAD_DMA_WS : K_WGRAD_DMA, q.flops, st);
  note_launch(WS ? K_WGRAD_DMA_WS : K_WGRAD_DMA);
  return launch_lds<wgrad_dma_kernel<NSTG, 4, WS>>(dim3(grid), dim3(WS ? 8 * 64 : 256), LDSB, st, q);
}
static int launch_wgrad_dma(const WgradParams& p, const WgradPlan& pl, hipStream_t st) {
  WgradParams q = p;
  q.gx = pl.gx; q.gy = pl.gy; q.gz = pl.Z;
  const int grid = pl.gx * pl.gy * pl.Z;
  if (g_wgrad_ws) return launch_wgrad_dma_t<3, true>(q, grid, st);
  return launch_wgrad_dma_t<2, false>(q, grid, st);
}

template <class P>
static int launch_wgrad_p(const WgradParams& p, const WgradPlan& pl, int nsub, hipStream_t st) {
  if (g_wgrad_dma && p.big_bytes && p.s_bytes && !P::IS_F32 && pl.BG == 128 && pl.BS == 128 && nsub == 1 && !p.big_row_elems && p.logCb >= 6 && p.logCb < 30 &&
      pl.mchunk % WGD_BKP == 0 && p.logOW <= 6 &&
      ((1 << p.logOHW) <= WGD_BKP || p.H == p.sy * ((1 << p.logOHW) >> p.logOW)))
    return launch_wgrad_dma(p, pl, st);
  if (pl.BG == 128 && pl.BS == 128 && nsub == 1) return launch_wgrad_t<P, 128, 128, 1>(p, pl, st);
  if (pl.BG == 128 && pl.BS == 64 && nsub == 1) return launch_wgrad_t<P, 128, 64, 1>(p, pl, st);
  if (pl.BG == 64 && pl.BS == 64 && nsub == 2) return launch_wgrad_t<P, 64, 64, 2>(p, pl, st);
  if (pl.BG == 64 && pl.BS == 64 && nsub == 1) return launch_wgrad_t<P, 64, 64, 1>(p, pl, st);
  JCK_FAIL(JCK_E_ARG, "wgrad: unsupported tile plan");
}

static int run_wgrad(int prec, WgradParams& p, const WgradPlan& pl, int nsub, float* ws, size_t ws_bytes, hipStream_t st) {
  if (ws_bytes < pl.ws) JCK_FAIL(JCK_E_WS, "wgrad: workspace too small: need " + std::to_string(pl.ws));
  p.part = ws; p.CsRows = pl.CsRows; p.ncols = pl.ncols; p.mchunk = pl.mchunk;
  DISPATCH_P(prec, launch_wgrad_p<P>(p, pl, nsub, st));
}

static int launch_wgrad_reduce(const float* ws, int Z, int CsRows, int ncols, int Cs, int Cb, int logCbPad, float* grad,
                               int accumulate, hipStream_t st) {
  if (Cb % 64 == 0 && (1 << logCbPad) == Cb) {
    if (Z >= 16 && (long long)(Cb / 64) * Cs <= 1024)
      hipLaunchKernelGGL(wgrad_reduce16_kernel<4>, dim3(Cb / 64, Cs), dim3(1024), 0, st, ws, Z, CsRows, ncols, Cb, logCbPad, grad, accumulate);
    else
      hipLaunchKernelGGL(wgrad_reduce16_kernel<1>, dim3(Cb / 64, Cs), dim3(256), 0, st, ws, Z, CsRows, ncols, Cb, logCbPad, grad, accumulate);
  } else if (logCbPad == 2 && ncols == 64) {
    hipLaunchKernelGGL(wgrad_reduce_img_kernel, dim3(Cs), dim3(256), 0, st, ws, Z, CsRows, Cb, grad, accumulate);
  } else {
    const long long total = (long long)Cs * Cb * 16;
    hipLaunchKernelGGL(wgrad_reduce_kernel, dim3((unsigned)std::min<long long>((total + 255) / 256, 4096)), dim3(256), 0, st, ws,
                       Z, CsRows, ncols, Cs, Cb, logCbPad, 16, grad, accumulate);
  }
  HIPCHK(hipGetLastError());
  return JCK_OK;
}

extern "C" size_t jck_conv_wgrad_ws_bytes(int N, int Hb, int Wb, int Cb, int Cs) {
  const long long M = (long long)N * (Hb / 2) * (Wb / 2);
  return plan_wgrad(M, 16 * jck_pad_chan(Cb), Cs).ws;
}

extern "C" int jck_conv_wgrad(int prec, const void* small_side, const void* big_side, float* ws, size_t ws_bytes,
                              float* grad, int accumulate, int N, int Hb, int Wb, int Cb, int Cs, void* stream) {
  const int cbp = jck_pad_chan(Cb);
  if (!is_pow2(cbp) || !is_pow2(Hb) || !is_pow2(Wb) || Cs % 8 != 0) JCK_FAIL(JCK_E_ARG, "conv_wgrad: bad shape");
  const int OH = Hb / 2, OW = Wb / 2;
  WgradParams p = {};
  p.sside = small_side; p.big = big_side; p.Mtot = N * OH * OW; p.CsStride = Cs; p.logCb = ilog2(cbp);
  p.H = Hb; p.W = Wb; p.logOW = ilog2(OW); p.logOHW = ilog2(OH * OW); p.sy = p.sx = 2; p.ntaps = 16;
  for (int t = 0; t < 16; ++t) { p.dy[t] = (signed char)(t / 4 - 1); p.dx[t] = (signed char)(t % 4 - 1); }
  p.flops = 2.0 * p.Mtot * Cs * 16.0 * Cb;
  {
    const long long esz = prec_f32_storage(prec) ? 4 : 2;
    const long long bb = (long long)N * Hb * Wb * cbp * esz, sbytes = (long long)p.Mtot * Cs * esz;
    if (bb < (1ll << 31) && sbytes < (1ll << 31)) { p.big_bytes = (unsigned)bb; p.s_bytes = (unsigned)sbytes; }
  }
  const WgradPlan pl = plan_wgrad(p.Mtot, 16 * cbp, Cs);
  JCK_TRY(run_wgrad(prec, p, pl, cbp == 4 ? 2 : 1, ws, ws_bytes, (hipStream_t)stream));
  JCK_TRY(launch_wgrad_reduce(ws, pl.Z, pl.CsRows, pl.ncols, Cs, Cb, p.logCb, grad, accumulate, (hipStream_t)stream));
  return JCK_OK;
}

extern "C" size_t jck_g1_wgrad_ws_bytes(int B, int CiPad, int Co) { return plan_wgrad(B, 16 * Co, CiPad).ws; }

extern "C" int jck_g1_wgrad(int prec, const void* z, const void* dy, float* ws, size_t ws_bytes, float* grad,
                            int accumulate, int B, int Ci, int CiPad, int Co, void* stream) {
  if (!is_pow2(Co) || CiPad % 64 != 0) JCK_FAIL(JCK_E_ARG, "g1_wgrad: bad shape");
  WgradParams p = {};
  p.sside = z; p.big = dy; p.Mtot = B; p.CsStride = CiPad; p.logCb = ilog2(Co);
  p.H = 4; p.W = 4; p.logOW = 0; p.logOHW = 0; p.sy = p.sx = 1; p.ntaps = 16;
  for (int t = 0; t < 16; ++t) { p.dy[t] = (signed char)(t / 4); p.dx[t] = (signed char)(t % 4); }
  const WgradPlan pl = plan_wgrad(B, 16 * Co, CiPad);
  p.flops = 2.0 * B * Ci * 16.0 * Co;
  {
    const long long esz = prec_f32_storage(prec) ? 4 : 2;
    p.big_bytes = (unsigned)((long long)B * 16 * Co * esz); p.s_bytes = (unsigned)((long long)B * CiPad * esz);
  }
  int rc = run_wgrad(prec, p, pl, 1, ws, ws_bytes, (hipStream_t)stream);
  if (rc) return rc;
  JCK_TRY(launch_wgrad_reduce(ws, pl.Z, pl.CsRows, pl.ncols, Ci, Co, p.logCb, grad, accumulate, (hipStream_t)stream));
  return JCK_OK;
}

extern "C" int jck_head_unpack_grad(const float* dwp, int C, float* grad, int accumulate, void* stream) {
  return launch_wgrad_reduce(dwp, 1, 1, 16 * C, 1, C, ilog2(C), grad, accumulate, (hipStream_t)stream);
}

extern "C" int jck_linear_fwd(int prec, const void* x, const void* wp, const float* bias, void* out, int B, int Kpad, int N,
                              int NStore, int ksplit, void* stream) {
  if (Kpad % 64 || NStore % 4) JCK_FAIL(JCK_E_ARG, "linear_fwd: Kpad % 64 or NStore % 4");
  const int rows = jck_pad_rows(N);
// ... 52 lines not shown
```

jck-generation_amd/csrc/thin.hpp:

```cpp
#pragma once
#include "common.hpp"

struct ImgDownParams {
  const void* x;
  const void* w;
  void* out;
  float* stats;
  int ngroups;
  int H, W, logOH, logG;
  unsigned x_bytes;
};

template <int GPW>
static __global__ __launch_bounds__(256) void img_down_kernel(const ImgDownParams p) {
  __shared__ float red[4][128];
  const int lane = threadIdx.x & 63, wave = threadIdx.x >> 6;
  const int pcol = lane & 15, g = lane >> 4;
  const auto rs = make_rsrc(p.x, p.x_bytes);
  const bf16_t* wp = reinterpret_cast<const bf16_t*>(p.w);
  bf16x8 wf[4][2];
#pragma unroll
  for (int t = 0; t < 4; ++t) {
    const int c = 32 * (t >> 1) + 8 * (pcol >> 2) + 4 * (t & 1) + (pcol & 3);
#pragma unroll
    for (int s = 0; s < 2; ++s) wf[t][s] = *reinterpret_cast<const bf16x8*>(wp + c * 64 + s * 32 + g * 8);
  }
  const int OH = 1 << p.logOH, OW = 16 << p.logG;
  const int g0 = (blockIdx.x * 4 + wave) * GPW;
  u32x2 xr[GPW][2][2];
#pragma unroll
  for (int i = 0; i < GPW; ++i) {
    const int gi = g0 + i;
    const int ox = ((gi & ((1 << p.logG) - 1)) << 4) + pcol;
    const int row = gi >> p.logG;
    const int oy = row & (OH - 1), n = row >> p.logOH;
    const int ix = 2 * ox + 2 * (g & 1) - 1;
#pragma unroll
    for (int s = 0; s < 2; ++s) {
      const int iy = 2 * oy + 2 * s + (g >> 1) - 1;
      const bool oky = gi < p.ngroups && (unsigned)iy < (unsigned)p.H;
      const unsigned off = (unsigned)(((n * p.H + iy) * p.W + ix) * 8);
      xr[i][s][0] = __builtin_amdgcn_raw_buffer_load_b64(rs, (int)((oky && ix >= 0) ? off : JCK_OOB), 0, 0);
      xr[i][s][1] = __builtin_amdgcn_raw_buffer_load_b64(rs, (int)((oky && ix + 1 < p.W) ? off + 8u : JCK_OOB), 0, 0);
    }
  }
  float ssum[16], ssq[16];
#pragma unroll
  for (int k = 0; k < 16; ++k) { ssum[k] = 0.f; ssq[k] = 0.f; }
  bf16_t* outp = reinterpret_cast<bf16_t*>(p.out);
#pragma unroll
  for (int i = 0; i < GPW; ++i) {
    const int gi = g0 + i;
    f32x4 acc[4];
#pragma unroll
    for (int t = 0; t < 4; ++t) acc[t] = f32x4{0.f, 0.f, 0.f, 0.f};
#pragma unroll
    for (int s = 0; s < 2; ++s) {
      const u32x4 raw = {xr[i][s][0][0], xr[i][s][0][1], xr[i][s][1][0], xr[i][s][1][1]};
      const bf16x8 b = __builtin_bit_cast(bf16x8, raw);
#pragma unroll
      for (int t = 0; t < 4; ++t) acc[t] = mfma16(wf[t][s], b, acc[t]);
    }
    u32x4 o0, o1;
#pragma unroll
    for (int t = 0; t < 4; ++t) {
#pragma unroll
      for (int j = 0; j < 4; ++j) { const float v = acc[t][j]; ssum[4 * t + j] += v; ssq[4 * t + j] += v * v; }
    }
    o0[0] = pack2bf(acc[0][0], acc[0][1]); o0[1] = pack2bf(acc[0][2], acc[0][3]);
    o0[2] = pack2bf(acc[1][0], acc[1][1]); o0[3] = pack2bf(acc[1][2], acc[1][3]);
    o1[0] = pack2bf(acc[2][0], acc[2][1]); o1[1] = pack2bf(acc[2][2], acc[2][3]);
    o1[2] = pack2bf(acc[3][0], acc[3][1]); o1[3] = pack2bf(acc[3][2], acc[3][3]);
    if (gi < p.ngroups) {
      bf16_t* d = outp + ((long long)gi * 16 + pcol) * 64 + 8 * g;
      *reinterpret_cast<u32x4*>(d) = o0;
      *reinterpret_cast<u32x4*>(d + 32) = o1;
    }
  }
  if (!p.stats) return;
#pragma unroll
  for (int k = 0; k < 16; ++k) { ssum[k] = row16_sum(ssum[k]); ssq[k] = row16_sum(ssq[k]); }
  if (pcol == 0) {
#pragma unroll
    for (int k = 0; k < 16; ++k) {
      const int c = 32 * (k >> 3) + 8 * g + (k & 7);
      red[wave][c] = ssum[k]; red[wave][64 + c] = ssq[k];
    }
  }
  __syncthreads();
  if (threadIdx.x < 128) {
    const float t = red[0][threadIdx.x] + red[1][threadIdx.x] + red[2][threadIdx.x] + red[3][threadIdx.x];
    p.stats[(long long)blockIdx.x * 128 + threadIdx.x] = t;
  }
}

struct ImgUpParams {
  const void* a;
  const void* w;
  void* out;
  int nunits;
  int Hs, Ws, logYB, logG;
  unsigned a_bytes;
  int epi_tanh;
  const void* mul_t; float mul_scale;
};

#define IMGUP_WLD 584

__device__ __forceinline__ u32x4 dpp_from_left(u32x4 edge, u32x4 src) {
  u32x4 r;
#pragma unroll
  for (int k = 0; k < 4; ++k) r[k] = (unsigned)__builtin_amdgcn_update_dpp((int)edge[k], (int)src[k], 0x111, 0xf, 0xf, false);
  return r;
}
__device__ __forceinline__ u32x4 dpp_from_right(u32x4 edge, u32x4 src) {
  u32x4 r;
#pragma unroll
  for (int k = 0; k < 4; ++k) r[k] = (unsigned)__builtin_amdgcn_update_dpp((int)edge[k], (int)src[k], 0x101, 0xf, 0xf, false);
  return r;
}

template <int R>
static __global__ __launch_bounds__(256) void img_up_kernel(const ImgUpParams p) {
  __shared__ __attribute__((aligned(16))) bf16_t wl[16 * IMGUP_WLD];
  const int lane = threadIdx.x & 63, wave = threadIdx.x >> 6;
  const int pcol = lane & 15, g = lane >> 4;
  {
    const u32x4* src = reinterpret_cast<const u32x4*>(p.w);
    for (int c = threadIdx.x; c < 16 * 72; c += 256) {
      const int r = c / 72, q = c - r * 72;
      *reinterpret_cast<u32x4*>(wl + r * IMGUP_WLD + q * 8) = src[c];
    }
  }
  __syncthreads();
  const int unit = blockIdx.x * 4 + wave;
  if (unit >= p.nunits) return;
  const auto rs = make_rsrc(p.a, p.a_bytes);
  const int Hs = p.Hs, Ws = p.Ws;
  const int x0 = (unit & ((1 << p.logG) - 1)) << 4;
  const int yb = (unit >> p.logG) & ((1 << p.logYB) - 1), n = unit >> (p.logG + p.logYB);
  const int y0 = yb * R, x = x0 + pcol;
  bf16_t* outp = reinterpret_cast<bf16_t*>(p.out);
  const bf16_t* wrow = wl + pcol * IMGUP_WLD + g * 8;
  const int xh = pcol == 0 ? x0 - 1 : (pcol == 15 ? x0 + 16 : -1);
  const bool okh = (unsigned)xh < (unsigned)Ws;

  struct Row { u32x4 c[2], l[2], r[2]; };
  auto load_row = [&](int yy, u32x4 (&c)[2], u32x4 (&h)[2]) {
    const bool oky = (unsigned)yy < (unsigned)Hs;
    const unsigned base = (unsigned)(((n * Hs + yy) * Ws) * 128 + g * 16);
    const unsigned oc = oky ? base + (unsigned)x * 128u : JCK_OOB;
    const unsigned oh = (oky && okh) ? base + (unsigned)xh * 128u : JCK_OOB;
    c[0] = __builtin_amdgcn_raw_buffer_load_b128(rs, (int)oc, 0, 0);
    c[1] = __builtin_amdgcn_raw_buffer_load_b128(rs, (int)(oc + 64u), 0, 0);
    h[0] = __builtin_amdgcn_raw_buffer_load_b128(rs, (int)oh, 0, 0);
    h[1] = __builtin_amdgcn_raw_buffer_load_b128(rs, (int)(oh + 64u), 0, 0);
  };
  u32x4 rc[R + 2][2], rh[R + 2][2];
  constexpr int AHEAD = 4;
#pragma unroll
  for (int j = 0; j < AHEAD && j < R + 2; ++j) load_row(y0 - 1 + j, rc[j], rh[j]);
  Row win[3];
  auto shift_in = [&](int j, Row& w) {
#pragma unroll
    for (int h = 0; h < 2; ++h) {
      w.c[h] = rc[j][h];
      w.l[h] = dpp_from_left(rh[j][h], rc[j][h]);
      w.r[h] = dpp_from_right(rh[j][h], rc[j][h]);
    }
  };
  shift_in(0, win[0]);
  shift_in(1, win[1]);
#pragma unroll
  for (int i = 0; i < R; ++i) {
    if (i + AHEAD < R + 2) load_row(y0 - 1 + i + AHEAD, rc[i + AHEAD], rh[i + AHEAD]);
    shift_in(i + 2, win[(i + 2) % 3]);
    f32x4 acc = {0.f, 0.f, 0.f, 0.f};
#pragma unroll
    for (int d = 0; d < 3; ++d) {
      const Row& w = win[(i + d) % 3];
#pragma unroll
      for (int h = 0; h < 2; ++h) {
        acc = mfma16(lds_frag(wrow + ((d * 3 + 0) * 2 + h) * 32), __builtin_bit_cast(bf16x8, w.l[h]), acc);
        acc = mfma16(lds_frag(wrow + ((d * 3 + 1) * 2 + h) * 32), __builtin_bit_cast(bf16x8, w.c[h]), acc);
        acc = mfma16(lds_frag(wrow + ((d * 3 + 2) * 2 + h) * 32), __builtin_bit_cast(bf16x8, w.r[h]), acc);
      }
    }
    float v[4] = {acc[0], acc[1], acc[2], acc[3]};
    if (p.epi_tanh) {
#pragma unroll
      for (int r = 0; r < 4; ++r) v[r] = tanhf(v[r]);
    }
    const int y = y0 + i;
    const long long o = (((long long)n * 2 * Hs + 2 * y + (g >> 1)) * 2 * Ws + 2 * x + (g & 1)) * 4;
    if (p.mul_t) {
      float t[4];
      ld4(reinterpret_cast<const bf16_t*>(p.mul_t) + o, t);
#pragma unroll
      for (int r = 0; r < 4; ++r) v[r] = p.mul_scale * bf2f(f2bf(v[r])) * (1.f - t[r] * t[r]);
    }
    st4(outp + o, v);
  }
}
```

jck-generation_amd/csrc/wgrad.hpp:

```cpp
#pragma once
#include "common.hpp"

struct WgradParams {
  const void* sside;
  const void* big;
  float* part;
  int Mtot;
  int CsStride;
  int CsRows;
  int ncols;
  int logCb;
  int H, W;
  int logOW, logOHW;
  int sy, sx;
  int ntaps;
  signed char dy[16], dx[16];
  int mchunk;
  int big_row_elems;
  int gx, gy, gz;
  unsigned big_bytes, s_bytes;
  double flops;
};

#define WG_BKP 32
// ... 126 lines not shown
  const int trow = (lane >> 4) * 8 + ((lane & 15) >> 2), tcol = (lane & 3) * 4;
  for (int kc = 0; kc < nk; ++kc) {
    const bool more = kc + 1 < nk;
    if (more) load_tiles(mz0 + (kc + 1) * WG_BKP);
    if constexpr (SPLIT) {
      const bf16_t* gt = reinterpret_cast<const bf16_t*>(smem_raw + (kc & 1) * C::BUF_BYTES);
      const bf16_t* st = gt + WG_BKP * LDG;
      bf16x8 ah[FM], al[FM], bh[FN], bl[FN];
#pragma unroll
      for (int i = 0; i < FM; ++i) {
        const bf16_t* q = gt + trow * LDG + wg * FM * 16 + i * 16 + tcol;
        ah[i] = join_tr(lds_tr4(q), lds_tr4(q + 4 * LDG));
        al[i] = join_tr(lds_tr4(q + C::PLANE), lds_tr4(q + C::PLANE + 4 * LDG));
      }
#pragma unroll
      for (int j = 0; j < FN; ++j) {
        const bf16_t* q = st + trow * LDSS + ws * FN * 16 + j * 16 + tcol;
        bh[j] = join_tr(lds_tr4(q), lds_tr4(q + 4 * LDSS));
        bl[j] = join_tr(lds_tr4(q + C::PLANE), lds_tr4(q + C::PLANE + 4 * LDSS));
      }
#pragma unroll
      for (int i = 0; i < FM; ++i)
#pragma unroll
        for (int j = 0; j < FN; ++j) acc[i][j] = mfma16(al[i], bh[j], acc[i][j]);
#pragma unroll
      for (int i = 0; i < FM; ++i)
#pragma unroll
        for (int j = 0; j < FN; ++j) acc[i][j] = mfma16(ah[i], bl[j], acc[i][j]);
#pragma unroll
      for (int i = 0; i < FM; ++i)
#pragma unroll
        for (int j = 0; j < FN; ++j) acc[i][j] = mfma16(ah[i], bh[j], acc[i][j]);
    } else if constexpr (!F32) {
      const T* gt = reinterpret_cast<const T*>(smem_raw + (kc & 1) * C::BUF_BYTES);
      const T* st = gt + WG_BKP * LDG;
      bf16x8 a[FM], b[FN];
#pragma unroll
      for (int i = 0; i < FM; ++i) {
        const bf16_t* q = gt + trow * LDG + wg * FM * 16 + i * 16 + tcol;
        a[i] = join_tr(lds_tr4(q), lds_tr4(q + 4 * LDG));
      }
#pragma unroll
      for (int j = 0; j < FN; ++j) {
        const bf16_t* q = st + trow * LDSS + ws * FN * 16 + j * 16 + tcol;
        b[j] = join_tr(lds_tr4(q), lds_tr4(q + 4 * LDSS));
      }
#pragma unroll
      for (int i = 0; i < FM; ++i)
#pragma unroll
        for (int j = 0; j < FN; ++j) acc[i][j] = mfma16(a[i], b[j], acc[i][j]);
    } else {
      const T* gt = reinterpret_cast<const T*>(smem_raw + (kc & 1) * C::BUF_BYTES);
      const T* st = gt + WG_BKP * LDG;
      const float* ga = gt + (lane >> 4) * LDG + wg * FM * 16 + (lane & 15);
      const float* sb = st + (lane >> 4) * LDSS + ws * FN * 16 + (lane & 15);
#pragma unroll 4
      for (int kk = 0; kk < WG_BKP / 4; ++kk) {
        float a[FM], b[FN];
#pragma unroll
        for (int i = 0; i < FM; ++i) a[i] = ga[kk * 4 * LDG + i * 16];
#pragma unroll
        for (int j = 0; j < FN; ++j) b[j] = sb[kk * 4 * LDSS + j * 16];
#pragma unroll
        for (int i = 0; i < FM; ++i)
#pragma unroll
          for (int j = 0; j < FN; ++j) acc[i][j] = __builtin_amdgcn_mfma_f32_16x16x4f32(a[i], b[j], acc[i][j], 0, 0, 0);
      }
    }
    if (more) store_tiles((kc + 1) & 1);
    __syncthreads();
  }

  float* part = p.part + (long long)blockIdx.z * p.CsRows * p.ncols;
#pragma unroll
  for (int j = 0; j < FN; ++j) {
    const int cs = s0 + ws * FN * 16 + j * 16 + (lane & 15);
    if (cs >= p.CsRows) continue;
#pragma unroll
    for (int i = 0; i < FM; ++i) {
      const int col = g0 + wg * FM * 16 + i * 16 + (lane >> 4) * 4;
      if (col >= p.ncols) continue;
      *reinterpret_cast<f32x4*>(part + (long long)cs * p.ncols + col) = acc[i][j];
    }
  }
}

static __global__ void wgrad_reduce_kernel(const float* __restrict__ part, int Z, int CsRows, int ncols, int Cs, int Cb,
                                           int logCbPad, int ntaps, float* __restrict__ grad, int accumulate) {
  const long long total = (long long)Cs * Cb * ntaps;
  for (long long i = blockIdx.x * (long long)blockDim.x + threadIdx.x; i < total; i += (long long)gridDim.x * blockDim.x) {
    const int t = (int)(i % ntaps);
    const long long r = i / ntaps;
    const int cb = (int)(r % Cb);
    const int cs = (int)(r / Cb);
    const long long src = (long long)cs * ncols + ((long long)t << logCbPad) + cb;
    float s = 0.f;
    for (int z = 0; z < Z; ++z) s += part[(long long)z * CsRows * ncols + src];
    grad[i] = accumulate ? grad[i] + s : s;
  }
}

static __global__ __launch_bounds__(256) void wgrad_reduce_img_kernel(const float* __restrict__ part, int Z, int CsRows, int Cb,
                                                                      float* __restrict__ grad, int accumulate) {
  __shared__ float red[16][64];
  const int cs = blockIdx.x, c4 = (threadIdx.x & 15) * 4, zl = threadIdx.x >> 4;
  f32x4 s = {0.f, 0.f, 0.f, 0.f};
#pragma unroll 4
  for (int z = zl; z < Z; z += 16) s += *reinterpret_cast<const f32x4*>(part + ((long long)z * CsRows + cs) * 64 + c4);
#pragma unroll
  for (int k = 0; k < 4; ++k) red[zl][c4 + k] = s[k];
  __syncthreads();
  if (threadIdx.x < 64) {
    const int col = threadIdx.x, t = col >> 2, cb = col & 3;
    if (cb < Cb) {
      float v = 0.f;
#pragma unroll
      for (int k = 0; k < 16; ++k) v += red[k][col];
      float* d = grad + ((long long)cs * Cb + cb) * 16 + t;
      *d = accumulate ? *d + v : v;
    }
  }
}

template <int ZG>
static __global__ __launch_bounds__(256 * ZG) void wgrad_reduce16_kernel(const float* __restrict__ part, int Z, int CsRows, int ncols,
                                                                         int Cb, int logCbPad, float* __restrict__ grad,
                                                                         int accumulate) {
  __shared__ float tile[64][17];
  __shared__ f32x4 zsum[ZG > 1 ? ZG - 1 : 1][256];
  const int cs = blockIdx.y, cb0 = blockIdx.x * 64;
  const int tid = threadIdx.x & 255, zq = threadIdx.x >> 8;
  const int t = tid >> 4, c4 = (tid & 15) * 4;
  const float* src = part + (long long)cs * ncols + ((long long)t << logCbPad) + cb0 + c4;
  f32x4 s = {0.f, 0.f, 0.f, 0.f};
  for (int z = zq; z < Z; z += ZG) s += *reinterpret_cast<const f32x4*>(src + (long long)z * CsRows * ncols);
  if constexpr (ZG > 1) {
    if (zq > 0) zsum[zq - 1][tid] = s;
    __syncthreads();
    if (zq == 0) {
#pragma unroll
      for (int q = 0; q < ZG - 1; ++q) s += zsum[q][tid];
    }
  }
  if (zq == 0) {
#pragma unroll
    for (int k = 0; k < 4; ++k) tile[c4 + k][t] = s[k];
  }
  __syncthreads();
  if (zq != 0) return;
  const int cbl = tid >> 2, t4 = (tid & 3) * 4;
  float* dst = grad + ((long long)cs * Cb + cb0 + cbl) * 16 + t4;
  f32x4 o = {tile[cbl][t4], tile[cbl][t4 + 1], tile[cbl][t4 + 2], tile[cbl][t4 + 3]};
  if (accumulate) o += *reinterpret_cast<const f32x4*>(dst);
  *reinterpret_cast<f32x4*>(dst) = o;
}

static __device__ __attribute__((aligned(16))) unsigned int g_jck_zero_page_w[64];

#define WGD_BKP 64
template <int NSTG, int NW, bool WS = false>
static __global__ __launch_bounds__(WS ? 8 * 64 : NW * 64) void wgrad_dma_kernel(const WgradParams p) {
  static_assert(!WS || (NW == 4 && NSTG == 3), "wave specialisation: 4 loader + 4 consumer waves, 3 LDS stages");
  constexpr int BG = 128, BS = 128, FM = 4, FN = NW == 8 ? 2 : 4;
  constexpr int NQ = 16 / NW;
  constexpr int SW = 128 / (NW / 2);
  constexpr int ROWB = 256;
// ... 218 lines not shown
```

jck-generation_amd/hipgan/_lib.py:

```python
import ctypes as C
import os

import torch

HERE = os.path.dirname(os.path.abspath(__file__))
LIB_PATH = os.path.join(os.path.dirname(HERE), "lib", "libjckgan_hip.so")
PREC_BF16, PREC_F32, PREC_BF16X3 = 0, 1, 2

vp, i32, i64, f32, f64, sz = C.c_void_p, C.c_int, C.c_longlong, C.c_float, C.c_double, C.c_size_t


class StepInputs(C.Structure):
    _fields_ = [("real_nchw", vp), ("noise_real", vp), ("z", vp), ("noise_fake", vp), ("alpha", vp),
                ("lr", f32), ("grad_scale", f32), ("step", i32), ("labels", vp), ("drop_mask", vp * 4),
                ("real_u8", vp), ("real_idx", vp)]


PROTOS = {
    "jck_last_error": (C.c_char_p, []),
    "jck_last_launch": (C.c_char_p, []),
    "jck_launch_name": (C.c_char_p, [i32]),
    "jck_version": (i32, []),
    "jck_pad_rows": (i32, [i32]),
    "jck_pad_chan": (i32, [i32]),
    "jck_packed_bytes": (sz, [i32, i64]),
    "jck_stats_floats": (sz, [i64, i32, i32]),
    "jck_pack_down": (i32, [i32, vp, i32, i32, vp, vp]),
    "jck_pack_up": (i32, [i32, vp, i32, i32, vp, vp]),
    "jck_pack_g1": (i32, [i32, vp, i32, i32, i32, vp, vp]),
    "jck_pack_head": (i32, [vp, i32, vp, vp]),
    "jck_conv_down": (i32, [i32, vp, vp, vp, vp, C.POINTER(i32), i32, i32, i32, i32, i32, vp]),
    "jck_conv_up": (i32, [i32, vp, vp, vp, vp, C.POINTER(i32), i32, i32, i32, i32, i32, i32, vp]),
    "jck_conv_wgrad_ws_bytes": (sz, [i32, i32, i32, i32, i32]),
    "jck_conv_wgrad": (i32, [i32, vp, vp, vp, sz, vp, i32, i32, i32, i32, i32, i32, vp]),
    "jck_g1_fwd": (i32, [i32, vp, vp, vp, vp, C.POINTER(i32), i32, i32, i32, vp]),
    "jck_conv_up_affine": (i32, [i32, vp, vp, vp, vp, vp, i32, i32, i32, i32, i32, vp]),
    "jck_g1_fwd_affine": (i32, [i32, vp, vp, vp, vp, vp, i32, i32, i32, vp]),
    "jck_conv_down_mask": (i32, [i32, vp, vp, vp, vp, vp, i32, i32, i32, i32, i32, vp]),
    "jck_conv_down_affine": (i32, [i32, vp, vp, vp, vp, f32, vp, i32, i32, i32, i32, i32, vp]),
    "jck_conv_up_mask": (i32, [i32, vp, vp, vp, vp, f32, vp, i32, i32, i32, i32, i32, vp]),
    "jck_leaky_affine_bwd": (i32, [i32, vp, vp, vp, f32, vp, i64, i32, vp]),
    "jck_critic_ds": (i32, [vp, i32, f32, i32, vp, vp, vp]),
    "jck_latent_loss_ex": (i32, [i32, vp, vp, vp, vp, vp, vp, i32, i32, vp]),
    "jck_score_head": (i32, [i32, vp, vp, vp, i32, i32, vp, vp, vp]),
    "jck_latent_loss": (i32, [i32, vp, vp, vp, vp, i32, i32, vp]),
    "jck_latent_adam": (i32, [i32, vp, i32, i32, vp, vp, vp, f32, f32, i32, vp, i32, i32, vp]),
    "jck_bn_eval_aux": (i32, [i32, C.POINTER(vp), C.POINTER(vp), C.POINTER(vp), C.POINTER(vp), C.POINTER(vp), C.POINTER(i32), f32, vp]),
    "jck_img_to_u8": (i32, [i32, vp, vp, i32, i32, vp]),
    "jck_g1_wgrad_ws_bytes": (sz, [i32, i32, i32]),
    "jck_g1_wgrad": (i32, [i32, vp, vp, vp, sz, vp, i32, i32, i32, i32, i32, vp]),
    "jck_bn_finalize": (i32, [vp, i32, f32, vp, vp, vp, vp, vp, f32, f32, vp, i32, vp]),
    "jck_bn_act_fwd": (i32, [i32, vp, vp, f32, vp, i64, i32, vp]),
    "jck_bn_bwd_ws_floats": (sz, [i32]),
    "jck_bn_act_bwd": (i32, [i32, vp, vp, vp, f32, vp, vp, vp, vp, i64, i32, vp]),
    "jck_bn_finalize_grouped": (i32, [vp, i32, f32, vp, vp, f32, vp, vp, i32, i32, vp]),
    "jck_bn_act_fwd_grouped": (i32, [i32, vp, vp, f32, vp, i64, i32, i32, vp]),
    "jck_bn_fwd": (i32, [i32, vp, vp, i32, f32, vp, vp, f32, f32, vp, vp, vp, vp, vp, vp, f32, i64, i32, i32, vp]),
    "jck_conv_down_grouped": (i32, [i32, vp, vp, vp, vp, vp, i32, i32, i32, i32, i32, i32, vp]),
    "jck_conv_up_grouped": (i32, [i32, vp, vp, vp, vp, vp, i32, i32, i32, i32, i32, i32, vp]),
    "jck_bn_act_bwd_grouped": (i32, [i32, vp, vp, vp, f32, vp, vp, vp, vp, i64, i32, i32, i32, vp]),
    "jck_grid_sync_bytes": (sz, []),
    "jck_grid_sync_error": (i32, [vp]),
    "jck_bn_act_bwd_res": (i32, [i32, vp, vp, vp, f32, vp, vp, vp, vp, i64, i32, i32, i32, vp, vp]),
    "jck_img_prep": (i32, [i32, vp, vp, f32, f32, vp, i32, i32, vp]),
    "jck_resize_norm": (i32, [vp, vp, i32, i32, i32, i32, i32, i32, f32, f32, vp, vp, vp]),
    "jck_img_prep_u8": (i32, [i32, vp, vp, vp, f32, f32, vp, vp, i32, i32, i32, vp]),
    "jck_nhwc4_to_nchw": (i32, [i32, vp, vp, i32, i32, vp]),
    "jck_axpy_noise": (i32, [i32, vp, vp, f32, f32, vp, i32, i32, vp]),
    "jck_interp": (i32, [i32, vp, vp, vp, vp, i32, i32, vp]),
    "jck_mix_interp": (i32, [i32, vp, vp, vp, i32, f32, f32, vp, vp, vp, vp, i32, i32, vp]),
    "jck_gp_norm": (i32, [i32, vp, i32, i32, vp, i32, i32, vp, vp]),
    "jck_tanh_bwd": (i32, [i32, vp, vp, f32, vp, i64, vp]),
    "jck_head_fwd": (i32, [i32, vp, vp, vp, i32, i32, f32, i32, vp, vp, vp, i32, i32, i32, vp]),
    "jck_head_fwd_grouped": (i32, [i32, vp, vp, vp, i32, i32, i32, vp, vp, vp, vp, vp, vp, vp, i32, vp]),
    "jck_head_bwd_ws_floats": (sz, [i32]),
    "jck_pack_linear": (i32, [i32, vp, i32, i32, i32, i32, i32, i32, i32, vp, vp]),
    "jck_linear_fwd": (i32, [i32, vp, vp, vp, vp, i32, i32, i32, i32, i32, vp]),
    "jck_linear_finish": (i32, [i32, vp, i32, vp, vp, f32, vp, vp, i32, i32, vp]),
    "jck_linear_wgrad_ws_bytes": (sz, [i32, i32, i32]),
    "jck_linear_wgrad": (i32, [i32, vp, i32, vp, i32, vp, sz, vp, i32, i32, i32, vp]),
    "jck_unperm_linear_grad": (i32, [vp, i32, i32, i32, i32, i32, vp, i32, vp]),
    "jck_label_embed_fwd": (i32, [i32, vp, vp, vp, f32, i32, i32, i32, vp, i32, i32, vp, vp]),
    "jck_label_embed_bwd": (i32, [i32, vp, i32, i32, vp, vp, f32, i32, i32, i32, vp, vp, vp]),
    "jck_label_embed_fwd_tiled": (i32, [i32, vp, vp, vp, f32, i32, i32, i32, vp, i32, i32, vp, i32, vp]),
    "jck_label_embed_bwd_tiled": (i32, [i32, vp, i32, i32, vp, vp, f32, i32, i32, i32, vp, vp, i32, vp]),
    "jck_concat_rows": (i32, [i32, vp, i32, vp, i32, i32, vp]),
    "jck_split_rows": (i32, [i32, vp, i32, i32, vp, i32, vp]),
    "jck_dropout": (i32, [i32, vp, vp, f32, vp, i64, vp]),
    "jck_colsum": (i32, [i32, vp, i32, i32, i32, vp, vp]),
    "jck_sum_vec": (i32, [vp, i32, vp, vp]),
    "jck_cgan_z": (i32, [i32, vp, vp, i32, i32, i32, i32, vp, vp]),
    "jck_gp_grad": (i32, [i32, vp, vp, f32, i32, i32, vp, vp]),
    "jck_gp_head2": (i32, [i32, vp, vp, vp, i32, i32, vp, vp, vp, vp]),
    "jck_gp_head2_conv_ws_floats": (sz, [i32]),
    "jck_gp_head2_conv": (i32, [i32, vp, vp, vp, vp, i32, i32, vp, vp, vp, vp, vp]),
    "jck_bn2_ws_floats": (sz, [i32]),
    "jck_bn2_vchain": (i32, [i32, vp, vp, vp, vp, vp, vp, f32, vp, vp, vp, vp, i64, i32, vp]),
    "jck_bn2_reverse": (i32, [i32, vp, vp, vp, vp, vp, vp, f32, vp, vp, vp, vp, i64, i32, vp]),
    "jck_head_bwd": (i32, [i32, vp, vp, vp, i32, i32, vp, vp, i32, vp, vp]),
    "jck_head_unpack_grad": (i32, [vp, i32, vp, i32, vp]),
    "jck_head_bwd_conv": (i32, [i32, vp, vp, vp, i32, i32, vp, vp, vp, vp]),
    "jck_head_bwd_conv2": (i32, [i32, vp, vp, vp, i32, i32, i32, vp, vp, vp, vp]),
    "jck_adam": (i32, [vp, vp, vp, vp, i64, f64, f64, f64, f64, i32, f32, vp]),
    "jck_adam_ema": (i32, [vp, vp, vp, vp, vp, i64, f64, f64, f64, f64, i32, f32, f32, vp, vp]),
    "jck_engine_create": (i32, [C.POINTER(vp), i32, i32, i32]),
    "jck_engine_create_sized": (i32, [C.POINTER(vp), i32, i32, i32, i32]),
    "jck_engine_create_ex": (i32, [C.POINTER(vp), i32, i32, i32, i32, C.c_uint]),
    "jck_engine_image_size": (i32, [vp]),
    "jck_engine_num_tensors_of": (i32, [vp, i32]),
    "jck_engine_tensor_info_of": (i32, [vp, i32, i32, C.c_char_p, i32, C.POINTER(i32), C.POINTER(i64), C.POINTER(i64),
                                        C.POINTER(i32)]),
    "jck_engine_arena_numel_of": (i64, [vp, i32, i32]),
    "jck_engine_destroy": (None, [vp]),
    "jck_engine_num_tensors": (i32, [i32, i32]),
    "jck_engine_tensor_info": (i32, [i32, i32, i32, C.c_char_p, i32, C.POINTER(i32), C.POINTER(i64), C.POINTER(i64),
                                     C.POINTER(i32)]),
    "jck_engine_workspace_bytes": (sz, [vp]),
    "jck_engine_arena_numel": (i64, [i32, i32, i32]),
    "jck_engine_bind": (i32, [vp, vp, sz] + [vp] * 12),
    "jck_engine_repack": (i32, [vp, i32, vp]),
    "jck_engine_phase": (i32, [vp, i32, C.POINTER(StepInputs), vp]),
    "jck_engine_order_after_tail": (i32, [vp, vp]),
    "jck_engine_drop_prefetch": (i32, [vp, vp]),
    "jck_engine_grad_tail": (i64, [vp, i32]),
    "jck_engine_check": (i32, [vp]),
    "jck_engine_scalars": (vp, [vp]),
    "jck_engine_scalars_at": (vp, [vp, i32]),
    "jck_engine_sample": (i32, [vp, vp, vp, i32, vp, vp]),
    "jck_engine_sample_ex": (i32, [vp, vp, vp, i32, C.c_uint, vp, vp, vp]),
    "jck_engine_latent_grad": (i32, [vp, vp, vp, vp, i32, vp, vp, vp]),
    "jck_engine_project": (i32, [vp, vp, vp, vp, i32, i32, f32, f32, vp, vp, i32, vp, vp]),
    "jck_engine_latent_grad_ex": (i32, [vp, vp, vp, vp, vp, i32, f32, i32, vp, vp, vp, vp, vp]),
    "jck_engine_project_ex": (i32, [vp, vp, vp, vp, i32, i32, f32, f32, vp, i32, f32, vp, vp, i32, vp, vp, vp]),
    "jck_engine_score": (i32, [vp, vp, vp, vp, i32, vp, vp, vp]),
    "jck_engine_tensor": (vp, [vp, C.c_char_p, C.POINTER(i64)]),
    "jck_debug_tr_read": (i32, [vp, i32, vp, vp]),
    "jck_tune": (i32, [C.c_char_p, i32]),
    "jck_conv2d_nhwc_f32": (i32, [vp, vp, vp, vp, vp] + [i32] * 14 + [vp]),
    "jck_pool2d_nhwc_f32": (i32, [vp, vp] + [i32] * 10 + [vp]),
    "jck_global_avgpool_nhwc_f32": (i32, [vp, vp, i32, i32, i32, vp]),
    "jck_nchw_to_nhwc_f32": (i32, [vp, vp, i32, i32, i32, i32, vp]),
    "jck_mean_cov_f64": (i32, [vp, vp, vp, i32, i32, vp]),
    "jck_pairstat_ws_bytes": (sz, [i32, i32]),
    "jck_poly3_sum_f64": (i32, [vp, i32, vp, i32, i32, f64, f64, i32, vp, vp, vp]),
    "jck_knn_radius2_f32": (i32, [vp, i32, i32, i32, vp, vp]),
    "jck_manifold_hit_u8": (i32, [vp, i32, vp, vp, i32, i32, vp, vp]),
    "jck_knn_index_ws_bytes": (sz, [i32, i32]),
    "jck_knn_index_f32": (i32, [vp, i32, vp, i32, i32, i32, i64, i64, i32, i32, vp, vp, vp, vp]),
    "jck_engine_set_step": (i32, [vp, i32, f32, vp]),
    "jck_engine_bind_ema": (i32, [vp, vp]),
    "jck_engine_set_ema": (i32, [vp, f64, i32]),
    "jck_engine_graph_nodes": (i32, [vp]),
    "jck_engine_set_noise_seed": (i32, [vp, C.c_ulonglong]),
    "jck_step_rng": (i32, [vp, i32, C.c_ulonglong, vp, C.c_longlong, vp, C.c_longlong, vp, C.c_longlong, f32, vp]),
    "jck_img_prep_rng": (i32, [i32, vp, vp, i32, f32, f32, vp, i32, i32, vp]),
    "jck_img_prep_u8_rng": (i32, [i32, vp, vp, vp, i32, f32, f32, vp, i32, i32, i32, vp]),
    "jck_axpy_noise_rng": (i32, [i32, vp, vp, i32, f32, f32, vp, i32, i32, vp]),
    "jck_engine_capture_begin": (i32, [vp, vp]),
    "jck_engine_capture_end": (i32, [vp, vp, C.POINTER(vp)]),
    "jck_engine_capture_abort": (i32, [vp, vp]),
    "jck_graph_launch": (i32, [vp, vp]),
    "jck_graph_destroy": (None, [vp]),
    "jck_comm_unique_id": (i32, [vp]),
    "jck_comm_create": (i32, [C.POINTER(vp), vp, i32, i32]),
    "jck_comm_world": (i32, [vp]),
    "jck_comm_allreduce_enqueue": (i32, [vp, vp, sz, vp, C.POINTER(i32)]),
    "jck_comm_wait": (i32, [vp, i32, vp]),
    "jck_comm_destroy": (i32, [vp]),
    "jck_prof_enable": (i32, [i32]),
    "jck_prof_collect": (i32, [i32, C.POINTER(C.c_char_p), C.POINTER(i32), C.POINTER(f64), C.POINTER(f64), C.POINTER(f64), C.POINTER(vp)]),
}


class JckError(RuntimeError):
    pass


_cdll = None


def load_library(path=None):
    global _cdll
    if _cdll is not None:
        return _cdll
    path = path or os.environ.get("JCKGAN_LIB", LIB_PATH)
    if not os.path.exists(path):
        raise JckError(f"{path} not found: build it with `python __graft_entry__.py build` "
                       f"(hipcc --offload-arch=gfx950); there is no CPU fallback")
    dll = C.CDLL(path)
    partial = os.environ.get("JCKGAN_ALLOW_PARTIAL") == "1"
    for name, (res, args) in PROTOS.items():
        if partial and not hasattr(dll, name):
            continue
        fn = getattr(dll, name)
        fn.restype, fn.argtypes = res, args
    if os.path.abspath(path) == os.path.abspath(LIB_PATH) and os.environ.get("JCKGAN_ALLOW_STALE") != "1":
        from . import build as _build
        want, got = _build.source_id(), dll.jck_version()
        if got != want:
            raise JckError(f"{path} was built from other sources than the ones beside it (jck_version {got}, sources {want}): "
                           f"rebuild with `python __graft_entry__.py build`")
    _cdll = dll
    return dll


def _arg(a):
    if a is None:
        return None
    if isinstance(a, torch.Tensor):
        return a.data_ptr()
    return a


class _Lib:

    def __getattr__(self, name):
        dll = load_library()
        fn = getattr(dll, name)

        def call(*args):
            for a in args:
                if isinstance(a, torch.Tensor):
                    if not a.is_cuda:
                        raise JckError(f"{name}: tensor argument is on {a.device}; the HIP path needs device memory")
                    if not a.is_contiguous():
                        raise JckError(f"{name}: non-contiguous tensor argument")
            r = fn(*[_arg(a) for a in args])
            if fn.restype is i32 and name not in ("jck_version", "jck_pad_rows", "jck_pad_chan", "jck_engine_num_tensors", "jck_prof_collect", "jck_grid_sync_error", "jck_comm_world", "jck_engine_graph_nodes") \
                    and r != 0:
                raise JckError(f"{name} failed ({r}): {dll.jck_last_error().decode()}")
            return r
        call.__name__ = name
        setattr(self, name, call)
        return call


lib = _Lib()


def cur_stream():
    return torch.cuda.current_stream().cuda_stream
```

jck-generation_amd/hipgan/engine.py:

```python
import ctypes as C
import os

import torch

from ._lib import PREC_BF16, PREC_BF16X3, PREC_F32, JckError, StepInputs, cur_stream, lib, load_library

(PHASE_D_LOSS, PHASE_D_GP, PHASE_D_STEP, PHASE_G_LOSS, PHASE_G_STEP, PHASE_D_REAL, PHASE_D_FAKE, PHASE_D_REAL_FWD, PHASE_D_LOSS_A,
 PHASE_D_LOSS_B) = range(10)
PHASE_LAZY_JOIN = 0x100
PHASE_GP_ONLY = 10
PHASE_NO_RESIDENT = 0x200
ENGINE_GP_BACKWARD = 1
_PREC = {"bf16": PREC_BF16, "f32": PREC_F32, "bf16x3": PREC_BF16X3, PREC_BF16: PREC_BF16, PREC_F32: PREC_F32,
         PREC_BF16X3: PREC_BF16X3}
SCALAR_NAMES = ("loss_d", "loss_g", "d_x", "d_gz1", "d_gz2", "gp", "loss_real", "loss_fake")


def _layout(handle, net):
    dll = load_library()
    out = []
    for i in range(dll.jck_engine_num_tensors_of(handle, net)):
        name = C.create_string_buffer(64)
        kind, off, numel = C.c_int(), C.c_longlong(), C.c_longlong()
        shape = (C.c_int * 4)()
# ... 836 lines not shown
            raise JckError(f"CGAN {what} needs one-hot int64 labels [n,100]")
        return labels.to(self.device, torch.int64).contiguous()

    def score(self, images, labels=None, noise=None):
        from .sampler import images_to_target
        x = images_to_target(images)
        n = x.shape[0]
        if x.shape[2] != self.size:
            raise JckError(f"score: images are {x.shape[2]}x{x.shape[2]}, this discriminator takes {self.size}x{self.size}")
        lab = self._score_labels("score", labels, n)
        nz = None
        if noise is not None:
            if tuple(noise.shape) != tuple(x.shape):
                raise JckError(f"score: noise must be shaped like the images {tuple(x.shape)}, got {tuple(noise.shape)}")
            nz = noise.to(self.device, torch.float32).contiguous()
        self._score_ready("score")
        x = x.to(self.device, torch.float32).contiguous()
        logit = torch.empty(n, dtype=torch.float32, device=self.device)
        prob = torch.empty(n, dtype=torch.float32, device=self.device)
        for lo, hi in chunk_plan(n, self.batch):
            lib.jck_engine_score(self._h, x[lo:hi], None if nz is None else nz[lo:hi], None if lab is None else lab[lo:hi], hi - lo,
                                 logit[lo:hi], prob[lo:hi], cur_stream())
        self._keep_score = (x, nz, lab)
        return logit, prob

    def score_latents(self, z, labels=None):
        n = z.shape[0]
        if n < 1:
            raise JckError("score_latents: z is empty")
        zc = z.to(self.device, torch.float32).contiguous().view(-1, 100)
        if zc.shape[0] != n:
            raise JckError("score_latents: z must be [n,100]")
        lab = self._score_labels("score_latents", labels, n)
        self._score_ready("score_latents")
        logit = torch.empty(n, dtype=torch.float32, device=self.device)
        prob = torch.empty(n, dtype=torch.float32, device=self.device)
        for lo, hi in chunk_plan(n, self.batch):
            lc = None if lab is None else lab[lo:hi]
            lib.jck_engine_sample_ex(self._h, zc[lo:hi], lc, hi - lo, SAMPLE_EVAL, None, None, cur_stream())
            lib.jck_engine_score(self._h, None, None, lc, hi - lo, logit[lo:hi], prob[lo:hi], cur_stream())
        self._keep_score = (zc, lab)
        return logit, prob

    def sample_scored(self, z, labels=None, out="float"):
        if out not in ("float", "uint8"):
            raise JckError(f"sample_scored: out must be 'float' or 'uint8', got {out!r}")
        n = z.shape[0]
        if n < 1:
            raise JckError("sample_scored: z is empty")
        zc = z.to(self.device, torch.float32).contiguous().view(-1, 100)
        if zc.shape[0] != n:
            raise JckError("sample_scored: z must be [n,100]")
        lab = self._score_labels("sample_scored", labels, n)
        self._score_ready("sample_scored")
        shape, dt = ((n, self.size, self.size, 3), torch.uint8) if out == "uint8" else ((n, 3, self.size, self.size), torch.float32)
        res = torch.empty(shape, dtype=dt, device=self.device)
        logit = torch.empty(n, dtype=torch.float32, device=self.device)
        prob = torch.empty(n, dtype=torch.float32, device=self.device)
        for lo, hi in chunk_plan(n, self.batch):
            lc = None if lab is None else lab[lo:hi]
            lib.jck_engine_sample_ex(self._h, zc[lo:hi], lc, hi - lo, SAMPLE_EVAL, res[lo:hi] if out == "float" else None,
                                     res[lo:hi] if out == "uint8" else None, cur_stream())
            lib.jck_engine_score(self._h, None, None, lc, hi - lo, logit[lo:hi], prob[lo:hi], cur_stream())
        self._keep_score = (zc, lab)
        return res, logit, prob

    def score_current(self, n, labels=None):
        if not 1 <= n <= self.batch:
            raise JckError(f"score_current: n must be in [1, {self.batch}]")
        lab = self._score_labels("score_current", labels, n)
        self._score_ready("score_current")
        logit = torch.empty(n, dtype=torch.float32, device=self.device)
        prob = torch.empty(n, dtype=torch.float32, device=self.device)
        lib.jck_engine_score(self._h, None, None, lab, n, logit, prob, cur_stream())
        self._keep_score = (lab,)
        return logit, prob

    def tensor(self, name):
        self.join()
        n = C.c_longlong()
        p = load_library().jck_engine_tensor(self._h, name.encode(), C.byref(n))
        if not p:
            raise KeyError(name)
        f32 = name in ("prob", "ds", "norms", "acc", "rs", "prob_gp")
        dt = torch.bfloat16 if (self.prec == PREC_BF16 and not f32) else torch.float32
        return self._ws_view(p, n.value, dt).clone()


SAMPLE_EVAL = 1
CRITIC_MODES = {None: 0, "nsgan": 1, "logit": 2}


def chunk_plan(n, batch):
    if n < 0 or batch < 1:
        raise JckError(f"chunk_plan: n >= 0 and batch >= 1, got {n}, {batch}")
    return [(lo, min(lo + batch, n)) for lo in range(0, n, batch)]


class CganEngine(DcganEngine):

    family = 1
```

Before: 161,000 images/sec.

## Fold GP gradient-norm reduction into image conv_up and add specialized image wgrad kernel

The input-gradient conv_up of the discriminator's first layer now also writes per-unit partial sums of squares for the gradient penalty when GP backward is off. The step tail reduces these partials into per-sample norms, so the separate gp_norm kernel and its re-read of the gradient image are no longer needed. A second, separate change routes the bf16 64x64 two-subtile wgrad plan for the image-side layer to a new buffer-load, double-buffered MFMA kernel. Any other layer that hits that plan now fails with an error instead of using the generic kernel.

```diff
diff --git a/include/jckgan.h b/include/jckgan.h
--- a/include/jckgan.h
+++ b/include/jckgan.h
@@ -102,6 +102,9 @@
 int jck_mix_interp(int prec, const void* x, const float* noise_nchw, const unsigned* rng, int tensor_id, float keep, float mix, void* out,
                    const void* real, const float* alpha, void* xhat, int N, int HW, void* stream);
 int jck_gp_norm(int prec, const void* g, int N, int HW, float* scal, int slot, int scal_ld, float* norms, void* stream);
+int jck_conv_up_sqsum_units(int prec, int Hs, int Ws, int Cs, int Cb);
+int jck_conv_up_sqsum(int prec, const void* small_in, const void* w, void* big_out, float* sq_part, int N, int Hs, int Ws, int Cs,
+                      int Cb, void* stream);
 int jck_tanh_bwd(int prec, const void* g, const void* y, float scale, void* out, long long numel, void* stream);
 int jck_head_fwd(int prec, const void* a4, const float* wp, const float* bias , int B, int K,
                  float target, int mode, float* prob, float* ds, float* scal, int slot_loss, int slot_p, int scal_ld, void* stream);
diff --git a/jck-generation_amd/csrc/engine.hip b/jck-generation_amd/csrc/engine.hip
--- a/jck-generation_amd/csrc/engine.hip
+++ b/jck-generation_amd/csrc/engine.hip
@@ -125,6 +125,7 @@
 static unsigned jck_event_flags() { return hipEventDisableTiming | hipEventDisableSystemFence; }
 struct StepState {
   bool gp_done = false;
+  bool gp_folded = false;
   bool gp_inflight = false;
   bool join_pending = false, mid_recorded = false;
   long long real_fwd_step = -1;
@@ -183,6 +184,8 @@
   float *acc, *scal_out;
   float *acc2, *scal2;
   int acc_ld = 0;
+  float *gp_sq, *gp_sq2;
+  int gp_units = 0;
   float *head_ws, *gp2_ws;
   float* hp2;
   unsigned long long noise_seed = 0x6a636b67616e0001ull;
@@ -265,6 +268,8 @@
     acc_ld = (B + 63) / 64 * 64;
     acc2 = c.take<float>((size_t)2 * 8 * acc_ld); scal2 = c.take<float>(16);
     acc = acc2; scal_out = scal2;
+    gp_units = jck_conv_up_sqsum_units(prec, TT.D_HB[0] / 2, TT.D_HB[0] / 2, TT.D_CS[0], TT.D_CB[0]);
+    gp_sq2 = c.take<float>((size_t)2 * B * std::max(gp_units, 1)); gp_sq = gp_sq2;
     hp2 = c.take<float>(16);
     for (int q = 0; q < 2; ++q) {
       rz[q] = c.take<float>((size_t)B * 100); ralpha[q] = c.take<float>((size_t)(B + 3) / 4 * 4);
@@ -646,10 +651,12 @@
   bool xgrad = false;
   XgradEpi* xe = nullptr;
   bool gp_norm = false;
+  bool gp_fold = false;
 };
 static int d_convs_backward(jck_engine* e, const DActs& S, const void* x_in, int B, hipStream_t st, const DBackward& o) {
   const int G = S.groups, gw = o.gw;
   hipStream_t side = gw > 0 ? o.side : nullptr;
+  const bool fold = o.gp_norm && o.gp_fold && o.xgrad && !o.xe && e->gp_units > 0;
   for (int i = TT.NS - 1; i >= 0; --i) {
     const int hb = TT.D_HB[i], cs = TT.D_CS[i], cb = TT.D_CB[i];
     const long long rows = (long long)B * (hb / 2) * (hb / 2);
@@ -681,10 +688,12 @@
     else if (o.xgrad) {
       const void* g0 = S.group(e, G - 1, 1).g[0];
       if (o.xe) JCK_TRY(conv_up_tanh_bwd_ev(e->prec, g0, e->d_up[0], o.xe->tanh_y, o.xe->scale, o.xe->out, B, hb / 2, hb / 2, cs, cb, st, o.xe->done, &o.xe->fused));
-      if (!o.xe || !o.xe->fused) JCK_TRY(jck_conv_up(e->prec, g0, e->d_up[0], S.gx, nullptr, nullptr, 0, B, hb / 2, hb / 2, cs, cb, st));
-    }
-  }
-  if (o.gp_norm) JCK_TRY(jck_gp_norm(e->prec, S.gx, B, TT.HW, e->acc, 6, e->acc_ld, S.norms, st));
+      if (fold) JCK_TRY(jck_conv_up_sqsum(e->prec, g0, e->d_up[0], S.gx, e->gp_sq, B, hb / 2, hb / 2, cs, cb, st));
+      else if (!o.xe || !o.xe->fused) JCK_TRY(jck_conv_up(e->prec, g0, e->d_up[0], S.gx, nullptr, nullptr, 0, B, hb / 2, hb / 2, cs, cb, st));
+    }
+  }
+  if (o.gp_norm && !fold) JCK_TRY(jck_gp_norm(e->prec, S.gx, B, TT.HW, e->acc, 6, e->acc_ld, S.norms, st));
+  if (o.gp_norm) e->ss.gp_folded = fold;
   if (side && o.join) {
     HIPCHK(hipEventRecord(e->evWdone, side));
     if (o.lazy_join) { e->ss.join_pending = true; e->ss.mid_recorded = false; }
@@ -704,6 +713,7 @@
   const int gw = G - 1;
   DBackward bw;
   bw.gw = gw; bw.side = side; bw.xgrad = bw.gp_norm = true; bw.part = part; bw.lazy_join = part == 1 && lazy_tail;
+  bw.gp_fold = !e->gp_bwd;
   if (part == 2) return d_convs_backward(e, S, x_in, B, st, bw);
   {
     float tg[4] = {0.f, 0.f, 0.f, 0.f};
@@ -1174,6 +1184,7 @@
     t.l[i].C = cs;
   }
   t.nl = TT.NS; t.npass = 4; t.momentum = BN_MOM; t.acc = e->acc; t.acc_ld = e->acc_ld; t.B = c.B; t.invB = 1.0f / (float)c.B; t.lambda_gp = 10.0f; t.out = e->scal_out;
+  if (e->ss.gp_folded) { t.gp_sq = e->gp_sq; t.gp_units = e->gp_units; }
   return repack_convs(e, 0, c.st, &t, cdiv(TT.G_C1, 256));
 }
 
@@ -1200,6 +1211,7 @@
     else if (e->hp_lr[q] != loc.lr) JCK_TRY(refresh_adam_scalars(e, loc.step, loc.lr, st));
   }
   e->acc = e->acc2 + (size_t)8 * e->acc_ld * e->parity;
+  e->gp_sq = e->gp_sq2 + (size_t)e->B * std::max(e->gp_units, 1) * e->parity;
   e->scal_out = e->scal2 + 8 * e->parity;
   return JCK_OK;
 }
@@ -1654,6 +1666,7 @@
   struct { const char* n; const void* p; long long c; } tab[] = {
       {"fake", e->fake, img}, {"fake_raw", e->fake_raw, img}, {"real_noisy", e->real_noisy, img}, {"xhat", e->xhat, img},
       {"d_gx", D.gx, img}, {"prob", D.prob, e->B}, {"ds", D.ds, e->B}, {"norms", D.norms, e->B}, {"acc", e->acc, (long long)8 * e->acc_ld},
+      {"gp_sq", e->gp_sq, (long long)e->B * e->gp_units},
       {"d_y1", D.y[0], (long long)e->B * (TT.S / 2) * (TT.S / 2) * 64}, {"d_a4", D.a[TT.NS - 1], (long long)e->B * TT.FEAT},
       {"g_y1", e->g_y[0], (long long)e->B * TT.FEAT}, {"g_a4", e->g_a[TT.NS - 1], (long long)e->B * (TT.S / 2) * (TT.S / 2) * 64}};
   for (auto& t : tab)
diff --git a/jck-generation_amd/csrc/ew_optim.hpp b/jck-generation_amd/csrc/ew_optim.hpp
--- a/jck-generation_amd/csrc/ew_optim.hpp
+++ b/jck-generation_amd/csrc/ew_optim.hpp
@@ -257,7 +257,8 @@
 }
 
 struct TailLayer { const float* rec; float* rm; float* rv; long long* nbt; int C; };
-struct TailJobs { TailLayer l[5]; int nl; int npass; float momentum; const float* acc; int acc_ld, B; float invB, lambda_gp; float* out; };
+struct TailJobs { TailLayer l[5]; int nl; int npass; float momentum; const float* acc; int acc_ld, B; float invB, lambda_gp; float* out;
+                  const float* gp_sq; int gp_units; };
 __device__ __forceinline__ void step_tail_block(const TailJobs& t, int bx, int by) {
   if (by == t.nl) {
     if (bx != 0) return;
@@ -266,7 +267,15 @@
 #pragma unroll
     for (int q = 0; q < 7; ++q) {
       float s = 0.f;
-      for (int n = threadIdx.x; n < t.B; n += 256) s += t.acc[(long long)q * t.acc_ld + n];
+      if (q == 6 && t.gp_sq) {
+        for (int n = threadIdx.x; n < t.B; n += 256) {
+          float ss = 0.f;
+          for (int u = 0; u < t.gp_units; ++u) ss += t.gp_sq[(long long)n * t.gp_units + u];
+          const float nr = sqrtf(ss);
+          s += (nr - 1.f) * (nr - 1.f);
+        }
+      } else
+        for (int n = threadIdx.x; n < t.B; n += 256) s += t.acc[(long long)q * t.acc_ld + n];
       tot[q] = block_sum256(s, sm);
     }
     if (threadIdx.x == 0) {
diff --git a/jck-generation_amd/csrc/ops_gemm.hip b/jck-generation_amd/csrc/ops_gemm.hip
--- a/jck-generation_amd/csrc/ops_gemm.hip
+++ b/jck-generation_amd/csrc/ops_gemm.hip
@@ -275,9 +275,9 @@
 }
 #define IMG_UP_R 8
 static int launch_img_up(const void* a, const void* w, void* out, int epi_tanh, int N, int Hs, int Ws, double flops, hipStream_t st,
-                         const void* mul_t = nullptr, float mul_scale = 1.f, hipEvent_t done = nullptr) {
+                         const void* mul_t = nullptr, float mul_scale = 1.f, hipEvent_t done = nullptr, float* sq_part = nullptr) {
   ImgUpParams q = {};
-  q.a = a; q.w = w; q.out = out; q.epi_tanh = epi_tanh; q.mul_t = mul_t; q.mul_scale = mul_scale;
+  q.a = a; q.w = w; q.out = out; q.epi_tanh = epi_tanh; q.mul_t = mul_t; q.mul_scale = mul_scale; q.sq_part = sq_part;
   q.nunits = N * (Hs / IMG_UP_R) * (Ws / 16); q.Hs = Hs; q.Ws = Ws; q.logYB = ilog2(Hs / IMG_UP_R); q.logG = ilog2(Ws / 16);
   q.a_bytes = (unsigned)((long long)N * Hs * Ws * 64 * 2);
   ProfScope prof(K_IMG_UP, flops, st);
@@ -394,6 +394,18 @@
   if (!*fused) return JCK_OK;
   return launch_img_up(small_in, w, out, 0, N, Hs, Ws, 2.0 * N * Hs * Ws * 4.0 * Cb * 4.0 * Cs, stream, tanh_y, scale, done);
 }
+extern "C" int jck_conv_up_sqsum_units(int prec, int Hs, int Ws, int Cs, int Cb) {
+  if (prec != JCK_PREC_BF16 || jck_pad_chan(Cb) != 4 || Cs != 64 || !is_pow2(Hs) || !is_pow2(Ws) || Ws % 16 || Hs % IMG_UP_R) return 0;
+  return (Hs / IMG_UP_R) * (Ws / 16);
+}
+extern "C" int jck_conv_up_sqsum(int prec, const void* small_in, const void* w, void* big_out, float* sq_part, int N, int Hs, int Ws,
+                                 int Cs, int Cb, void* stream) {
+  if (!small_in || !w || !big_out || !sq_part || N < 1) JCK_FAIL(JCK_E_ARG, "conv_up_sqsum: null tensor or N < 1");
+  if (!jck_conv_up_sqsum_units(prec, Hs, Ws, Cs, Cb)) JCK_FAIL(JCK_E_ARG, "conv_up_sqsum: bf16, Cs = 64 and a 3 / 4-channel output only");
+  if ((long long)N * Hs * Ws * 16 >= (1ll << 31)) JCK_FAIL(JCK_E_ARG, "conv_up_sqsum: tensor exceeds 2^31 elements");
+  return launch_img_up(small_in, w, big_out, 0, N, Hs, Ws, 2.0 * N * Hs * Ws * 4.0 * Cb * 4.0 * Cs, (hipStream_t)stream, nullptr, 1.f, nullptr,
+                       sq_part);
+}
 extern "C" int jck_conv_up(int prec, const void* small_in, const void* w, void* big_out, float* stats, int* stats_slots,
                            int epi_tanh, int N, int Hs, int Ws, int Cs, int Cb, void* stream) {
   return conv_up_impl(prec, small_in, w, big_out, stats, stats_slots, epi_tanh, N, Hs, Ws, Cs, Cb, stream);
@@ -490,6 +502,15 @@
   return launch_wgrad_dma_t<2, false>(q, grid, st);
 }
 
+static int launch_wgrad_img(const WgradParams& p, const WgradPlan& pl, hipStream_t st) {
+  constexpr KernelId id = kid_wgrad<PrecBf16, 64, 64, 2>();
+  ProfScope prof(id, p.flops, st);
+  note_launch(id);
+  hipLaunchKernelGGL(wgrad_img_kernel, dim3(1, pl.gy, pl.Z), dim3(256), 0, st, p);
+  HIPCHK(hipGetLastError());
+  return JCK_OK;
+}
+
 template <class P>
 static int launch_wgrad_p(const WgradParams& p, const WgradPlan& pl, int nsub, hipStream_t st) {
   if (g_wgrad_dma && p.big_bytes && p.s_bytes && !P::IS_F32 && pl.BG == 128 && pl.BS == 128 && nsub == 1 && !p.big_row_elems && p.logCb >= 6 && p.logCb < 30 &&
@@ -498,7 +519,14 @@
     return launch_wgrad_dma(p, pl, st);
   if (pl.BG == 128 && pl.BS == 128 && nsub == 1) return launch_wgrad_t<P, 128, 128, 1>(p, pl, st);
   if (pl.BG == 128 && pl.BS == 64 && nsub == 1) return launch_wgrad_t<P, 128, 64, 1>(p, pl, st);
-  if (pl.BG == 64 && pl.BS == 64 && nsub == 2) return launch_wgrad_t<P, 64, 64, 2>(p, pl, st);
+  if (pl.BG == 64 && pl.BS == 64 && nsub == 2) {
+    if constexpr (!P::IS_F32) {
+      if (pl.gx != 1 || p.ntaps != 16 || p.logCb != 2 || p.big_row_elems) JCK_FAIL(JCK_E_ARG, "wgrad: not an image-side layer");
+      return launch_wgrad_img(p, pl, st);
+    } else {
+      return launch_wgrad_t<P, 64, 64, 2>(p, pl, st);
+    }
+  }
   if (pl.BG == 64 && pl.BS == 64 && nsub == 1) return launch_wgrad_t<P, 64, 64, 1>(p, pl, st);
   JCK_FAIL(JCK_E_ARG, "wgrad: unsupported tile plan");
 }
diff --git a/jck-generation_amd/csrc/thin.hpp b/jck-generation_amd/csrc/thin.hpp
--- a/jck-generation_amd/csrc/thin.hpp
+++ b/jck-generation_amd/csrc/thin.hpp
@@ -103,6 +103,7 @@
   unsigned a_bytes;
   int epi_tanh;
   const void* mul_t; float mul_scale;
+  float* sq_part;
 };
 
 #define IMGUP_WLD 584
@@ -171,6 +172,7 @@
   };
   shift_in(0, win[0]);
   shift_in(1, win[1]);
+  float ssq = 0.f;
 #pragma unroll
   for (int i = 0; i < R; ++i) {
     if (i + AHEAD < R + 2) load_row(y0 - 1 + i + AHEAD, rc[i + AHEAD], rh[i + AHEAD]);
@@ -200,5 +202,13 @@
       for (int r = 0; r < 4; ++r) v[r] = p.mul_scale * bf2f(f2bf(v[r])) * (1.f - t[r] * t[r]);
     }
     st4(outp + o, v);
-  }
-}
+    if (p.sq_part) {
+#pragma unroll
+      for (int r = 0; r < 3; ++r) { const float q = bf2f(f2bf(v[r])); ssq += q * q; }
+    }
+  }
+  if (p.sq_part) {
+    ssq = wave_sum(ssq);
+    if (lane == 0) p.sq_part[unit] = ssq;
+  }
+}
diff --git a/jck-generation_amd/csrc/wgrad.hpp b/jck-generation_amd/csrc/wgrad.hpp
--- a/jck-generation_amd/csrc/wgrad.hpp
+++ b/jck-generation_amd/csrc/wgrad.hpp
@@ -232,6 +232,100 @@
       if (col >= p.ncols) continue;
       *reinterpret_cast<f32x4*>(part + (long long)cs * p.ncols + col) = acc[i][j];
     }
+  }
+}
+
+#define WGI_DEPTH 4
+static __global__ __launch_bounds__(256) void wgrad_img_kernel(const WgradParams p) {
+  constexpr int D = WGI_DEPTH, LD = 64 + 16;
+  static_assert(D % 2 == 0, "the LDS buffer of a k-step is its ring slot's parity");
+  __shared__ __attribute__((aligned(16))) bf16_t tiles[2][2][WG_BKP * LD];
+  const int tid = threadIdx.x, lane = tid & 63, wave = tid >> 6;
+  const int s0 = blockIdx.y * 64;
+  const int mz0 = blockIdx.z * p.mchunk;
+  const int mz1 = min(mz0 + p.mchunk, p.Mtot);
+  const int rows = max(mz1 - mz0, 0);
+  const int nk = (rows + WG_BKP - 1) / WG_BKP;
+  const int OHWm = (1 << p.logOHW) - 1, OWm = (1 << p.logOW) - 1;
+  const int n0 = mz0 >> p.logOHW;
+  const int nimg = rows ? ((mz1 - 1) >> p.logOHW) - n0 + 1 : 0;
+  const auto rs_s = make_rsrc(reinterpret_cast<const bf16_t*>(p.sside) + (long long)mz0 * p.CsStride,
+                              (unsigned)((long long)rows * p.CsStride * 2));
+  const auto rs_b = make_rsrc(reinterpret_cast<const bf16_t*>(p.big) + (((long long)n0 * p.H * p.W) << 2),
+                              (unsigned)(((long long)nimg * p.H * p.W) << 3));
+
+  const int gu = tid & 7, gr = tid >> 3;
+  const int dy0 = p.dy[2 * gu], dx0 = p.dx[2 * gu], dy1 = p.dy[2 * gu + 1], dx1 = p.dx[2 * gu + 1];
+  const bool scol = s0 + gu * 8 < p.CsStride;
+  const unsigned soff0 = (unsigned)((gr * p.CsStride + s0 + gu * 8) * 2), sstep = (unsigned)(WG_BKP * p.CsStride * 2);
+
+  u32x2 ga[D], gb[D];
+  u32x4 sv[D];
+  auto issue = [&](int slot, int kc) __attribute__((always_inline)) {
+    const int m = mz0 + kc * WG_BKP + gr;
+    const bool rok = m < mz1;
+    const int n = (m >> p.logOHW) - n0, rem = m & OHWm;
+    const int iy = (rem >> p.logOW) * p.sy, ix = (rem & OWm) * p.sx;
+    const int iya = iy + dy0, ixa = ix + dx0, iyb = iy + dy1, ixb = ix + dx1;
+    const bool oka = rok && (unsigned)iya < (unsigned)p.H && (unsigned)ixa < (unsigned)p.W;
+    const bool okb = rok && (unsigned)iyb < (unsigned)p.H && (unsigned)ixb < (unsigned)p.W;
+    const unsigned oa = (unsigned)(((n * p.H + iya) * p.W + ixa) << 3), ob = (unsigned)(((n * p.H + iyb) * p.W + ixb) << 3);
+    ga[slot] = __builtin_amdgcn_raw_buffer_load_b64(rs_b, (int)(oka ? oa : JCK_OOB), 0, 0);
+    gb[slot] = __builtin_amdgcn_raw_buffer_load_b64(rs_b, (int)(okb ? ob : JCK_OOB), 0, 0);
+    sv[slot] = __builtin_amdgcn_raw_buffer_load_b128(rs_s, (int)(scol ? soff0 + (unsigned)kc * sstep : JCK_OOB), 0, 0);
+  };
+  auto store = [&](int slot, int buf) __attribute__((always_inline)) {
+    *reinterpret_cast<u32x4*>(&tiles[buf][0][gr * LD + gu * 8]) = u32x4{ga[slot][0], ga[slot][1], gb[slot][0], gb[slot][1]};
+    *reinterpret_cast<u32x4*>(&tiles[buf][1][gr * LD + gu * 8]) = sv[slot];
+  };
+
+  const int wg = wave >> 1, ws = wave & 1;
+  f32x4 acc[2][2];
+#pragma unroll
+  for (int i = 0; i < 2; ++i)
+#pragma unroll
+    for (int j = 0; j < 2; ++j) acc[i][j] = f32x4{0.f, 0.f, 0.f, 0.f};
+  const int trow = (lane >> 4) * 8 + ((lane & 15) >> 2), tcol = (lane & 3) * 4;
+  auto compute = [&](int buf) __attribute__((always_inline)) {
+    bf16x8 a[2], b[2];
+#pragma unroll
+    for (int i = 0; i < 2; ++i) {
+      const bf16_t* q = &tiles[buf][0][trow * LD + wg * 32 + i * 16 + tcol];
+      a[i] = join_tr(lds_tr4(q), lds_tr4(q + 4 * LD));
+    }
+#pragma unroll
+    for (int j = 0; j < 2; ++j) {
+      const bf16_t* q = &tiles[buf][1][trow * LD + ws * 32 + j * 16 + tcol];
+      b[j] = join_tr(lds_tr4(q), lds_tr4(q + 4 * LD));
+    }
+#pragma unroll
+    for (int i = 0; i < 2; ++i)
+#pragma unroll
+      for (int j = 0; j < 2; ++j) acc[i][j] = mfma16(a[i], b[j], acc[i][j]);
+  };
+
+#pragma unroll
+  for (int j = 0; j < D; ++j) issue(j, j);
+  store(0, 0);
+  __syncthreads();
+  for (int kb = 0; kb < nk; kb += D) {
+#pragma unroll
+    for (int j = 0; j < D; ++j) {
+      issue(j, kb + j + D);
+      compute(j & 1);
+      store((j + 1) % D, (j + 1) & 1);
+      __syncthreads();
+    }
+  }
+
+  float* part = p.part + (long long)blockIdx.z * p.CsRows * p.ncols;
+#pragma unroll
+  for (int j = 0; j < 2; ++j) {
+    const int cs = s0 + ws * 32 + j * 16 + (lane & 15);
+    if (cs >= p.CsRows) continue;
+#pragma unroll
+    for (int i = 0; i < 2; ++i)
+      *reinterpret_cast<f32x4*>(part + (long long)cs * p.ncols + wg * 32 + i * 16 + (lane >> 4) * 4) = acc[i][j];
   }
 }
 
diff --git a/jck-generation_amd/hipgan/_lib.py b/jck-generation_amd/hipgan/_lib.py
--- a/jck-generation_amd/hipgan/_lib.py
+++ b/jck-generation_amd/hipgan/_lib.py
@@ -70,6 +70,8 @@
     "jck_interp": (i32, [i32, vp, vp, vp, vp, i32, i32, vp]),
     "jck_mix_interp": (i32, [i32, vp, vp, vp, i32, f32, f32, vp, vp, vp, vp, i32, i32, vp]),
     "jck_gp_norm": (i32, [i32, vp, i32, i32, vp, i32, i32, vp, vp]),
+    "jck_conv_up_sqsum_units": (i32, [i32, i32, i32, i32, i32]),
+    "jck_conv_up_sqsum": (i32, [i32, vp, vp, vp, vp, i32, i32, i32, i32, i32, vp]),
     "jck_tanh_bwd": (i32, [i32, vp, vp, f32, vp, i64, vp]),
     "jck_head_fwd": (i32, [i32, vp, vp, vp, i32, i32, f32, i32, vp, vp, vp, i32, i32, i32, vp]),
     "jck_head_fwd_grouped": (i32, [i32, vp, vp, vp, i32, i32, i32, vp, vp, vp, vp, vp, vp, vp, i32, vp]),
@@ -226,7 +228,7 @@
                     if not a.is_contiguous():
                         raise JckError(f"{name}: non-contiguous tensor argument")
             r = fn(*[_arg(a) for a in args])
-            if fn.restype is i32 and name not in ("jck_version", "jck_pad_rows", "jck_pad_chan", "jck_engine_num_tensors", "jck_prof_collect", "jck_grid_sync_error", "jck_comm_world", "jck_engine_graph_nodes") \
+            if fn.restype is i32 and name not in ("jck_version", "jck_pad_rows", "jck_pad_chan", "jck_conv_up_sqsum_units", "jck_engine_num_tensors", "jck_prof_collect", "jck_grid_sync_error", "jck_comm_world", "jck_engine_graph_nodes") \
                     and r != 0:
                 raise JckError(f"{name} failed ({r}): {dll.jck_last_error().decode()}")
             return r
diff --git a/jck-generation_amd/hipgan/engine.py b/jck-generation_amd/hipgan/engine.py
--- a/jck-generation_amd/hipgan/engine.py
+++ b/jck-generation_amd/hipgan/engine.py
@@ -942,7 +942,7 @@
         p = load_library().jck_engine_tensor(self._h, name.encode(), C.byref(n))
         if not p:
             raise KeyError(name)
-        f32 = name in ("prob", "ds", "norms", "acc", "rs", "prob_gp")
+        f32 = name in ("prob", "ds", "norms", "acc", "gp_sq", "rs", "prob_gp")
         dt = torch.bfloat16 if (self.prec == PREC_BF16 and not f32) else torch.float32
         return self._ws_view(p, n.value, dt).clone()
 
```

Measured after the change: 161,500 images/sec, median of 6. About the same (+0.3%).
